# aehogan/lammps-induced-dipole-polarization-pair-style

Hardware: AMD Instinct MI355X
Metric: atom-steps/sec (higher is better)
Workload: dtype f64

## Files before the change

### include/polar_mi355x.h

```cpp
#ifndef POLAR_MI355X_H
#define POLAR_MI355X_H

#ifdef __cplusplus
extern "C" {
#endif

#define POLAR_OK 0
#define POLAR_WARN_NOT_CONVERGED 1
#define POLAR_RETRY_STEP 2
#define POLAR_ERR_INPUT -1
#define POLAR_ERR_NO_DEVICE -2
#define POLAR_ERR_HIP -3
#define POLAR_ERR_UNSUPPORTED -4
#define POLAR_ERR_STATE -5

enum { POLAR_DAMP_EXPONENTIAL = 0, POLAR_DAMP_NONE = 1 };

typedef struct polar_handle polar_handle;

typedef struct {
  double cut_lj_global, cut_coul;
  double polar_precision, polar_damp, polar_gamma;
  int iterations_max, damping_type, zodid, fixed_iteration;
  int polar_gs, polar_gs_ranked, use_previous, debug;
// ... 12 lines not shown
#define POLAR_ACCEL_MAX 8

typedef struct {
  double eng_vdwl, eng_coul, eng_pol;
  double u_self, u_ef, u_dd;
  double virial[6];
  double rmin;
  double rms_dmu;
  int iterations;
  int sweeps;
  int status;
  int ncolors;
  double ms_total, ms_rank, ms_ljcoul, ms_static, ms_solve, ms_force, ms_list;
  long long dd_pairs;
  double ms_color_host;
  double ms_kspace;
  int nkvec;
} polar_result;

int polar_create(int device, polar_handle **out);
int polar_destroy(polar_handle *h);
const char *polar_last_error(const polar_handle *h);
const char *polar_last_warning(const polar_handle *h);
int polar_device_count(void);
const char *polar_kernel_version(void);

int polar_pair_settings(polar_handle *h, int narg, const char *const *arg);
int polar_pair_coeff(polar_handle *h, int ntypes, int narg, const char *const *arg);
int polar_pair_modify(polar_handle *h, int narg, const char *const *arg);
int polar_pair_init(polar_handle *h, double g_ewald, double qqrd2e, const double special_lj[4],
                    const double special_coul[4]);
double polar_pair_cut(const polar_handle *h, int itype, int jtype);
double polar_pair_single(const polar_handle *h, double qi, double qj, int itype, int jtype, double rsq,
                         double factor_coul, double factor_lj, double *fforce);
const void *polar_pair_extract(const polar_handle *h, const char *name, int *dim);
int polar_get_settings(const polar_handle *h, polar_settings *out);

int polar_restart_pack(const polar_handle *h, void *buf, int max_bytes);
int polar_restart_unpack(polar_handle *h, const void *buf, int nbytes);
#define POLAR_RESTART_HEADER_BYTES 12

int polar_set_settings(polar_handle *h, const polar_settings *s);
int polar_set_types(polar_handle *h, int ntypes, const double *lj1, const double *lj2, const double *lj3,
                    const double *lj4, const double *offset, const double *cut_ljsq, const double *cutsq);
int polar_set_coul(polar_handle *h, double g_ewald, double qqrd2e, const double special_lj[4],
                   const double special_coul[4], int ncoultablebits, int ncoulmask, int ncoulshiftbits,
                   double tabinnersq, const double *rtable, const double *drtable, const double *ftable,
                   const double *dftable, const double *ctable, const double *dctable, const double *etable,
                   const double *detable);

int polar_set_box(polar_handle *h, const double boxlo[3], const double prd[3], const double tilt[3],
                  const int periodic[3], int triclinic);
int polar_set_atoms(polar_handle *h, int nlocal, int nghost, const double *x, const double *q,
                    const double *alpha, const int *type, const int *molecule);
int polar_set_positions(polar_handle *h, int nlocal, int nghost, const double *x);
int polar_set_positions_range(polar_handle *h, int lo, int hi, const double *x);
int polar_set_neighbors(polar_handle *h, int inum, const int *ilist, const int *numneigh,
                        int *const *firstneigh);
int polar_set_neighbors_csr(polar_handle *h, int inum, const int *ilist, const int *numneigh,
                            const long long *firstneigh, const int *neigh);

int polar_set_newton(polar_handle *h, int newton_pair);

int polar_build_neighbors(polar_handle *h, const double *cutneighsq, const int *tag, const int *nspecial,
                          const int *special, int maxspecial, const int special_flag[4],
                          int exclude_molecule_intra);

int polar_compute(polar_handle *h, int eflag, int vflag, double *f, double *mu, double *ef_static,
                  polar_result *out);
int polar_compute_peratom(polar_handle *h, int eflag, int vflag, double *f, double *mu, double *ef_static,
                          double *eatom, double *vatom, polar_result *out);

int polar_get_debug_trace(polar_handle *h, double *u_polar, int max);

int polar_get_debug_forces(polar_handle *h, double *out6);

int polar_get_colors(polar_handle *h, int *color, int n);

int polar_set_colors(polar_handle *h, const int *color, int n);

int polar_compute_resident(polar_handle *h, int eflag, int vflag, polar_result *out);
void *polar_dev_ptr(polar_handle *h, const char *name);
int polar_download(polar_handle *h, const char *name, double *dst, long long n);
int polar_upload_mu(polar_handle *h, const double *mu, long long n);


int polar_set_stream(polar_handle *h, void *hip_stream);
int polar_set_row_range(polar_handle *h, int lo, int hi);
int polar_set_global_count(polar_handle *h, long long natoms);
int polar_set_list_style(polar_handle *h, int full);
int polar_step_begin(polar_handle *h, int eflag, int vflag);
int polar_step_sweep(polar_handle *h);
int polar_step_sweep_phase(polar_handle *h, int color, int part);
int polar_step_sweep_part(polar_handle *h, int part, int nparts);
int polar_step_sweep_end(polar_handle *h, const double *dev_global_change);
int polar_step_sweep_end_n(polar_handle *h, const double *dev_global_change, int count);
int polar_step_state(polar_handle *h, int *done, int *iterations, int *status);
int polar_step_finish(polar_handle *h, polar_result *out);
int polar_mu_gather(polar_handle *h, long long lo, long long hi, double *dev_dst);
int polar_mu_scatter(polar_handle *h, long long lo, long long hi, const double *dev_src);
int polar_mu_gather_idx(polar_handle *h, const int *dev_idx, long long n, double *dev_dst);
int polar_mu_scatter_idx(polar_handle *h, const int *dev_idx, long long n, const double *dev_src);
int polar_change_export(polar_handle *h, double *dev_dst);
int polar_step_mu_get(polar_handle *h, long long lo, long long hi, double *mu_host);
int polar_step_mu_put_idx(polar_handle *h, long long n, const int *idx_host, const double *mu_host);
int polar_step_change_get(polar_handle *h, double *sum);
int polar_step_sweep_end_host(polar_handle *h, double global_change);

#define POLAR_DIST_ID_BYTES 128
typedef struct polar_dist polar_dist;
int polar_dist_unique_id(void *id128);
int polar_dist_create(const void *id128, int rank, int nranks, int device, polar_dist **out);
int polar_dist_destroy(polar_dist *d);
const char *polar_dist_last_error(const polar_dist *d);
int polar_dist_comm_count(const polar_dist *d);
int polar_dist_set_cadence(polar_dist *d, int reduce_every, int check_every);
int polar_dist_set_schedule(polar_dist *d, int lag, int my_class, int nclasses);
int polar_dist_set_halo(polar_dist *d, polar_handle *h, int npeers, const int *peers, const int *send_count, const int *send_idx,
                        const int *recv_count, const int *recv_idx);
int polar_dist_set_ghosts(polar_dist *d, polar_handle *h, int nghost, const int *owner, const double *shift);
int polar_dist_positions(polar_dist *d, polar_handle *h);
int polar_dist_exchange(polar_dist *d, polar_handle *h);
int polar_dist_step(polar_dist *d, polar_handle *h, int eflag, int vflag, polar_result *out);
int polar_dist_local_result(const polar_dist *d, polar_result *out);
int polar_dist_counters(const polar_dist *d, int *exchanges, int *allreduces);
#define POLAR_DIST_PROF_PARTS 5
int polar_dist_profile(polar_dist *d, int enable);
int polar_dist_profile_get(const polar_dist *d, double *ms_by_part, int *intervals);

#ifdef __cplusplus
}
#endif
#endif
```

### lammps-induced-dipole-polarization-pair-style_amd/__init__.py

```python
from __future__ import annotations

import ctypes as C
import importlib
import os
import subprocess

import numpy as np

_HERE = os.path.dirname(os.path.abspath(__file__))
_CSRC = os.path.join(_HERE, "csrc")
LIB_PATH = os.path.join(_HERE, "libpolar_mi355x.so")
LIB_PATH_LAB = os.path.join(_HERE, "libpolar_mi355x_lab.so")
HIPCC = os.environ.get("HIPCC", "/opt/rocm/bin/hipcc")
HIP_FLAGS = ["--offload-arch=gfx950", "-O3", "-std=c++17", "-fPIC", "-shared"]

_lib = None
_lib_lab = None


class PolarError(RuntimeError):

    def __init__(self, code, message):
        super().__init__(message)
        self.code = code
# ... 14 lines not shown
def build(force=False, verbose=False, lab=True):
    from concurrent.futures import ThreadPoolExecutor

    jobs, links = [], []
    for path, extra, tag in ((LIB_PATH, [], "product"), (LIB_PATH_LAB, ["-DPOLAR_LAB"], "lab")):
        if path == LIB_PATH_LAB and not lab:
            continue
        stale = (not os.path.exists(path)) or any(os.path.getmtime(s) > os.path.getmtime(path) for s in _sources(lab=(path == LIB_PATH_LAB)))
        if not (force or stale):
            continue
        odir = os.path.join(_CSRC, "build", tag)
        os.makedirs(odir, exist_ok=True)
        objs = []
        for tu in TRANSLATION_UNITS:
            obj = os.path.join(odir, tu.replace(".hip", ".o"))
            objs.append(obj)
            jobs.append([HIPCC] + [f for f in HIP_FLAGS if f != "-shared"] + extra + ["-Wno-unused-function", "-c", "-o", obj, os.path.join(_CSRC, tu)])
        links.append([HIPCC, "--offload-arch=gfx950", "-fPIC", "-shared", "-o", path] + objs)

    def run(cmd):
        if verbose:
            print(" ".join(cmd), flush=True)
        subprocess.check_call(cmd)

    if jobs:
        with ThreadPoolExecutor(max_workers=min(len(jobs), max(1, (os.cpu_count() or 2)))) as ex:
            list(ex.map(run, jobs))
        for cmd in links:
            run(cmd)
    return LIB_PATH


class Settings(C.Structure):
    _fields_ = [("cut_lj_global", C.c_double), ("cut_coul", C.c_double), ("polar_precision", C.c_double),
                ("polar_damp", C.c_double), ("polar_gamma", C.c_double), ("iterations_max", C.c_int),
                ("damping_type", C.c_int), ("zodid", C.c_int), ("fixed_iteration", C.c_int), ("polar_gs", C.c_int),
                ("polar_gs_ranked", C.c_int), ("use_previous", C.c_int), ("debug", C.c_int), ("dd_cutoff", C.c_double),
                ("device_neigh", C.c_int), ("restart_polar", C.c_int), ("deterministic", C.c_int), ("polar_sor", C.c_double), ("rccl_halo", C.c_int), ("polar_accel", C.c_int),
                ("polar_ewald", C.c_double)]


class Result(C.Structure):
    _fields_ = [("eng_vdwl", C.c_double), ("eng_coul", C.c_double), ("eng_pol", C.c_double), ("u_self", C.c_double),
                ("u_ef", C.c_double), ("u_dd", C.c_double), ("virial", C.c_double * 6), ("rmin", C.c_double),
                ("rms_dmu", C.c_double), ("iterations", C.c_int), ("sweeps", C.c_int), ("status", C.c_int),
                ("ncolors", C.c_int), ("ms_total", C.c_double), ("ms_rank", C.c_double), ("ms_ljcoul", C.c_double),
                ("ms_static", C.c_double), ("ms_solve", C.c_double), ("ms_force", C.c_double), ("ms_list", C.c_double),
                ("dd_pairs", C.c_longlong), ("ms_color_host", C.c_double), ("ms_kspace", C.c_double), ("nkvec", C.c_int)]


_dp, _ip, _llp = C.POINTER(C.c_double), C.POINTER(C.c_int), C.POINTER(C.c_longlong)
_cpp = C.POINTER(C.c_char_p)
EXPORTS = {
    "polar_create": (C.c_int, [C.c_int, C.POINTER(C.c_void_p)]),
    "polar_destroy": (C.c_int, [C.c_void_p]),
    "polar_last_error": (C.c_char_p, [C.c_void_p]),
    "polar_last_warning": (C.c_char_p, [C.c_void_p]),
    "polar_device_count": (C.c_int, []),
    "polar_kernel_version": (C.c_char_p, []),
    "polar_pair_settings": (C.c_int, [C.c_void_p, C.c_int, _cpp]),
    "polar_pair_coeff": (C.c_int, [C.c_void_p, C.c_int, C.c_int, _cpp]),
    "polar_pair_modify": (C.c_int, [C.c_void_p, C.c_int, _cpp]),
    "polar_pair_init": (C.c_int, [C.c_void_p, C.c_double, C.c_double, _dp, _dp]),
    "polar_pair_cut": (C.c_double, [C.c_void_p, C.c_int, C.c_int]),
    "polar_pair_single": (C.c_double, [C.c_void_p, C.c_double, C.c_double, C.c_int, C.c_int, C.c_double, C.c_double,
                                       C.c_double, _dp]),
    "polar_pair_extract": (C.c_void_p, [C.c_void_p, C.c_char_p, _ip]),
    "polar_get_settings": (C.c_int, [C.c_void_p, C.POINTER(Settings)]),
    "polar_set_settings": (C.c_int, [C.c_void_p, C.POINTER(Settings)]),
    "polar_set_types": (C.c_int, [C.c_void_p, C.c_int] + [_dp] * 7),
    "polar_set_coul": (C.c_int, [C.c_void_p, C.c_double, C.c_double, _dp, _dp, C.c_int, C.c_int, C.c_int, C.c_double]
                       + [_dp] * 8),
    "polar_set_box": (C.c_int, [C.c_void_p, _dp, _dp, _dp, _ip, C.c_int]),
    "polar_set_atoms": (C.c_int, [C.c_void_p, C.c_int, C.c_int, _dp, _dp, _dp, _ip, _ip]),
    "polar_set_positions": (C.c_int, [C.c_void_p, C.c_int, C.c_int, _dp]),
    "polar_set_neighbors": (C.c_int, [C.c_void_p, C.c_int, _ip, _ip, C.POINTER(_ip)]),
    "polar_set_neighbors_csr": (C.c_int, [C.c_void_p, C.c_int, _ip, _ip, _llp, _ip]),
    "polar_build_neighbors": (C.c_int, [C.c_void_p, _dp, _ip, _ip, _ip, C.c_int, _ip, C.c_int]),
    "polar_compute": (C.c_int, [C.c_void_p, C.c_int, C.c_int, _dp, _dp, _dp, C.POINTER(Result)]),
    "polar_compute_peratom": (C.c_int, [C.c_void_p, C.c_int, C.c_int, _dp, _dp, _dp, _dp, _dp, C.POINTER(Result)]),
    "polar_compute_resident": (C.c_int, [C.c_void_p, C.c_int, C.c_int, C.POINTER(Result)]),
    "polar_dev_ptr": (C.c_void_p, [C.c_void_p, C.c_char_p]),
    "polar_download": (C.c_int, [C.c_void_p, C.c_char_p, _dp, C.c_longlong]),
    "polar_upload_mu": (C.c_int, [C.c_void_p, _dp, C.c_longlong]),
    "polar_set_stream": (C.c_int, [C.c_void_p, C.c_void_p]),
    "polar_set_row_range": (C.c_int, [C.c_void_p, C.c_int, C.c_int]),
    "polar_set_global_count": (C.c_int, [C.c_void_p, C.c_longlong]),
    "polar_step_mu_get": (C.c_int, [C.c_void_p, C.c_longlong, C.c_longlong, _dp]),
    "polar_step_mu_put_idx": (C.c_int, [C.c_void_p, C.c_longlong, _ip, _dp]),
    "polar_step_change_get": (C.c_int, [C.c_void_p, _dp]),
    "polar_step_sweep_end_host": (C.c_int, [C.c_void_p, C.c_double]),
    "polar_step_sweep_end_n": (C.c_int, [C.c_void_p, C.c_void_p, C.c_int]),
    "polar_set_list_style": (C.c_int, [C.c_void_p, C.c_int]),
    "polar_set_newton": (C.c_int, [C.c_void_p, C.c_int]),
    "polar_get_debug_trace": (C.c_int, [C.c_void_p, _dp, C.c_int]),
    "polar_get_debug_forces": (C.c_int, [C.c_void_p, _dp]),
    "polar_get_colors": (C.c_int, [C.c_void_p, C.POINTER(C.c_int), C.c_int]),
    "polar_restart_pack": (C.c_int, [C.c_void_p, C.c_void_p, C.c_int]),
    "polar_restart_unpack": (C.c_int, [C.c_void_p, C.c_void_p, C.c_int]),
    "polar_step_begin": (C.c_int, [C.c_void_p, C.c_int, C.c_int]),
    "polar_step_sweep": (C.c_int, [C.c_void_p]),
    "polar_step_sweep_part": (C.c_int, [C.c_void_p, C.c_int, C.c_int]),
    "polar_step_sweep_end": (C.c_int, [C.c_void_p, C.c_void_p]),
    "polar_step_state": (C.c_int, [C.c_void_p, _ip, _ip, _ip]),
    "polar_step_finish": (C.c_int, [C.c_void_p, C.POINTER(Result)]),
    "polar_mu_gather": (C.c_int, [C.c_void_p, C.c_longlong, C.c_longlong, C.c_void_p]),
    "polar_mu_scatter": (C.c_int, [C.c_void_p, C.c_longlong, C.c_longlong, C.c_void_p]),
    "polar_mu_gather_idx": (C.c_int, [C.c_void_p, C.c_void_p, C.c_longlong, C.c_void_p]),
    "polar_mu_scatter_idx": (C.c_int, [C.c_void_p, C.c_void_p, C.c_longlong, C.c_void_p]),
    "polar_change_export": (C.c_int, [C.c_void_p, C.c_void_p]),
    "polar_dist_unique_id": (C.c_int, [C.c_void_p]),
    "polar_dist_create": (C.c_int, [C.c_void_p, C.c_int, C.c_int, C.c_int, C.POINTER(C.c_void_p)]),
    "polar_dist_destroy": (C.c_int, [C.c_void_p]),
    "polar_dist_last_error": (C.c_char_p, [C.c_void_p]),
    "polar_dist_set_cadence": (C.c_int, [C.c_void_p, C.c_int, C.c_int]),
    "polar_dist_set_halo": (C.c_int, [C.c_void_p, C.c_void_p, C.c_int, _ip, _ip, _ip, _ip, _ip]),
    "polar_dist_set_schedule": (C.c_int, [C.c_void_p, C.c_int, C.c_int, C.c_int]),
    "polar_dist_set_ghosts": (C.c_int, [C.c_void_p, C.c_void_p, C.c_int, _ip, _dp]),
    "polar_dist_positions": (C.c_int, [C.c_void_p, C.c_void_p]),
    "polar_dist_local_result": (C.c_int, [C.c_void_p, C.POINTER(Result)]),
    "polar_dist_comm_count": (C.c_int, [C.c_void_p]),
    "polar_step_sweep_phase": (C.c_int, [C.c_void_p, C.c_int, C.c_int]),
    "polar_set_colors": (C.c_int, [C.c_void_p, _ip, C.c_int]),
    "polar_set_positions_range": (C.c_int, [C.c_void_p, C.c_int, C.c_int, _dp]),
    "polar_dist_exchange": (C.c_int, [C.c_void_p, C.c_void_p]),
    "polar_dist_step": (C.c_int, [C.c_void_p, C.c_void_p, C.c_int, C.c_int, C.POINTER(Result)]),
    "polar_dist_counters": (C.c_int, [C.c_void_p, _ip, _ip]),
    "polar_dist_profile": (C.c_int, [C.c_void_p, C.c_int]),
    "polar_dist_profile_get": (C.c_int, [C.c_void_p, _dp, _ip]),
}


def lib(lab=False):
    global _lib, _lib_lab
    if lab:
        if _lib_lab is None:
            if not os.path.exists(LIB_PATH_LAB):
                raise PolarError(-2, f"{LIB_PATH_LAB} is missing: run __graft_entry__.build()")
            lib()
            L = C.CDLL(LIB_PATH_LAB)
            for name, (res, args) in EXPORTS.items():
                fn = getattr(L, name)
                fn.restype, fn.argtypes = res, args
            _lib_lab = L
        return _lib_lab
    if _lib is None:
        if not os.path.exists(LIB_PATH):
            raise PolarError(-2, f"{LIB_PATH} is missing: run __graft_entry__.build() (hipcc, gfx950); "
                                 "there is no CPU fallback for the polarization hot path")
        try:
            import torch
        except ImportError:
            pass
        L = C.CDLL(LIB_PATH)
        for name, (res, args) in EXPORTS.items():
            fn = getattr(L, name)
            fn.restype, fn.argtypes = res, args
        _lib = L
    return _lib


def device_count():
    return lib().polar_device_count()


def kernel_version():
# ... 172 lines not shown
        if getattr(st, "polar_accel", 0):
            args += ["polar_accel", str(int(st.polar_accel))]
        if getattr(st, "polar_ewald", 0.0):
            args += ["polar_ewald", repr(float(st.polar_ewald))]
        self.settings(args)
        if modify_args:
            self.modify(list(modify_args))
        return args

    def set_system(self, sysm):
        self._ck(self.L.polar_set_newton(self.h, int(sysm.extra.get("newton_pair", 1))))
        self.set_box(sysm.boxlo, sysm.prd, tilt=getattr(sysm, "tilt", (0.0, 0.0, 0.0)),
                     triclinic=int(getattr(sysm, "triclinic", 0)))
        self.set_atoms(sysm.nlocal, sysm.nghost, sysm.x, sysm.q, sysm.alpha, sysm.type, sysm.molecule)
        self.set_neighbors_csr(sysm.ilist, sysm.numneigh, sysm.firstneigh, sysm.neigh)

    def build_neighbors(self, cutneighsq, tag=None, nspecial=None, special=None, special_flag=(1, 2, 2, 2),
                        exclude_molecule_intra=False):
        cn = np.ascontiguousarray(cutneighsq, dtype=np.float64)
        keep = [cn]
        ip = lambda a: None if a is None else (keep.append(np.ascontiguousarray(a, dtype=np.int32)) or
                                               keep[-1].ctypes.data_as(_ip))
        sf = np.ascontiguousarray(special_flag, dtype=np.int32)
        maxspecial = 0 if special is None else int(np.asarray(special).shape[1])
        self._ck(self.L.polar_build_neighbors(self.h, _dptr(cn), ip(tag), ip(nspecial), ip(special), maxspecial,
                                              sf.ctypes.data_as(_ip), int(bool(exclude_molecule_intra))))

    def build_neighbors_from_system(self, sysm, skin=None):
        wlm = importlib.import_module(__name__ + ".workload")
        w = sysm.ntypes + 1
        cutneigh = sysm.extra["cutneigh"] if skin is None else float(np.sqrt(sysm.tables["cutsq"][1:, 1:].max())) + skin
        cn = np.full((w, w), cutneigh * cutneigh)
        nsp = sp = None
        if sysm.extra.get("special"):
            nsp, sp = wlm.lammps_special_arrays(sysm.nlocal, sysm.extra["special"])
        tag = (np.asarray(sysm.owner) + 1).astype(np.int32)
        self.build_neighbors(cn, tag, nsp, sp, wlm.neighbor_special_flag(sysm.special_lj, sysm.special_coul),
                             sysm.extra.get("exclude_intra", False))

    def compute(self, eflag=1, vflag=2, mu=None, want_ef=True):
        n, nall = self.nlocal, self.nlocal + self.nghost
        f = np.zeros((nall, 3))
        mu = np.zeros((n, 3)) if mu is None else np.array(mu, dtype=np.float64, copy=True)
        ef = np.zeros((n, 3))
        res = Result()
        eatom = vatom = None
        if eflag // 2 or vflag // 4:
            eatom = np.zeros(nall) if eflag // 2 else None
            vatom = np.zeros((nall, 6)) if vflag // 4 else None
            rc = self._ck(self.L.polar_compute_peratom(
                self.h, eflag, vflag, _dptr(f), _dptr(mu), _dptr(ef) if want_ef else None,
                _dptr(eatom) if eatom is not None else None, _dptr(vatom) if vatom is not None else None,
                C.byref(res)))
        else:
            rc = self._ck(self.L.polar_compute(self.h, eflag, vflag, _dptr(f), _dptr(mu),
                                               _dptr(ef) if want_ef else None, C.byref(res)))
        out = _result_dict(res)
        out.update(f=f, mu=mu, ef_static=ef, status=rc, warning=self.L.polar_last_warning(self.h).decode(),
                   eatom=eatom, vatom=vatom)
        return out

    def compute_resident(self, eflag=1, vflag=2):
        res = Result()
        rc = self._ck(self.L.polar_compute_resident(self.h, eflag, vflag, C.byref(res)))
        out = _result_dict(res)
        out.update(status=rc, warning=self.L.polar_last_warning(self.h).decode())
        return out

    def debug_trace(self, nmax=1024):
        a = np.zeros(nmax)
        n = self._ck(self.L.polar_get_debug_trace(self.h, _dptr(a), nmax))
        return a[:n].copy()

    def debug_forces(self):
        a = np.zeros(6)
        self._ck(self.L.polar_get_debug_forces(self.h, _dptr(a)))
        return a[:3].copy(), a[3:].copy()

    def colors(self, n):
        a = np.full(n, -1, dtype=np.int32)
        nc = self._ck(self.L.polar_get_colors(self.h, a.ctypes.data_as(C.POINTER(C.c_int)), n))
        return nc, a

    def download(self, name, n):
        a = np.zeros(n)
        self._ck(self.L.polar_download(self.h, name.encode(), _dptr(a), n))
        return a


class PolarDist:

    @staticmethod
    def unique_id():
        buf = C.create_string_buffer(128)
        rc = lib().polar_dist_unique_id(buf)
        if rc < 0:
            raise PolarError(rc, "polar_dist_unique_id failed (is RCCL available?)")
        return buf.raw

    def __init__(self, unique_id, rank, nranks, device=0):
        self.L = lib()
        self.d = C.c_void_p()
        self.rank, self.nranks = rank, nranks
        rc = self.L.polar_dist_create(C.c_char_p(bytes(unique_id)), rank, nranks, device, C.byref(self.d))
        if rc < 0:
            raise PolarError(rc, self.L.polar_dist_last_error(self.d).decode())

    def _ck(self, rc):
        if rc < 0:
            raise PolarError(rc, self.L.polar_dist_last_error(self.d).decode())
        return rc

    def set_cadence(self, reduce_every=1, check_every=4):
        self._ck(self.L.polar_dist_set_cadence(self.d, reduce_every, check_every))

    def set_halo(self, pair, peers, send_lists, recv_lists):
        peers = np.ascontiguousarray(peers, dtype=np.int32)
        sc = np.array([len(a) for a in send_lists], dtype=np.int32)
        rc_ = np.array([len(a) for a in recv_lists], dtype=np.int32)
        si = np.ascontiguousarray(np.concatenate([np.asarray(a, dtype=np.int32) for a in send_lists]) if len(send_lists) else np.zeros(0, np.int32))
        ri = np.ascontiguousarray(np.concatenate([np.asarray(a, dtype=np.int32) for a in recv_lists]) if len(recv_lists) else np.zeros(0, np.int32))
        self._ck(self.L.polar_dist_set_halo(self.d, pair.h, len(peers), _iptr(peers), _iptr(sc), _iptr(si) if len(si) else None,
                                            _iptr(rc_), _iptr(ri) if len(ri) else None))

    def set_schedule(self, lag=1, my_class=0, nclasses=0):
        self._ck(self.L.polar_dist_set_schedule(self.d, lag, my_class, nclasses))

    def set_ghosts(self, pair, owner, shift):
        owner = np.ascontiguousarray(owner, dtype=np.int32)
        shift = np.ascontiguousarray(shift, dtype=np.float64)
        self._ck(self.L.polar_dist_set_ghosts(self.d, pair.h, len(owner), _iptr(owner) if len(owner) else None, _dptr(shift) if len(owner) else None))

    def positions(self, pair):
        self._ck(self.L.polar_dist_positions(self.d, pair.h))

    def local_result(self):
        res = Result()
        self._ck(self.L.polar_dist_local_result(self.d, C.byref(res)))
        return _result_dict(res)

    def comm_count(self):
        return self._ck(self.L.polar_dist_comm_count(self.d))

    PROFILE_PARTS = ("other", "sweep_kernels", "stop_rule", "exchange", "accel")

    def profile(self, enable=True):
        self._ck(self.L.polar_dist_profile(self.d, 1 if enable else 0))

    def profile_get(self):
        ms = (C.c_double * len(self.PROFILE_PARTS))()
        n = C.c_int()
        self._ck(self.L.polar_dist_profile_get(self.d, ms, C.byref(n)))
        out = {k: float(v) for k, v in zip(self.PROFILE_PARTS, ms)}
        out["intervals"] = n.value
        return out

    def exchange(self, pair):
        self._ck(self.L.polar_dist_exchange(self.d, pair.h))

    def step(self, pair, eflag=1, vflag=2):
        res = Result()
        rc = self._ck(self.L.polar_dist_step(self.d, pair.h, eflag, vflag, C.byref(res)))
        out = _result_dict(res)
        ex, ar = C.c_int(), C.c_int()
        self.L.polar_dist_counters(self.d, C.byref(ex), C.byref(ar))
        out.update(status=rc, warning=pair.L.polar_last_warning(pair.h).decode(), exchanges=ex.value, allreduces=ar.value)
# ... 38 lines not shown
```

### lammps-induced-dipole-polarization-pair-style_amd/csrc/lab/lists_cluster_rows.hpp

```cpp
struct ClusterRows {
  const int4 *members;
  int ncl;
};
static __global__ __launch_bounds__(POLAR_BLOCK) void k_cl_build(ClusterRows cl, const double4 *__restrict__ pos4, Box box,
                                                          CellGrid g, const long long *__restrict__ cell_first,
                                                          double ddcutsq, long long pitch, int *__restrict__ cnt,
                                                          int *__restrict__ dd_j, int pad_index,
                                                          int *__restrict__ wrapf, int *__restrict__ overflow,
                                                          unsigned long long *__restrict__ total) {
  const int lane = threadIdx.x & 63;
  const int c = blockIdx.x * POLAR_ROWS_PER_BLOCK + (threadIdx.x >> 6);
  if (c >= cl.ncl) return;
  const int4 mem = cl.members[c];
  const int m0 = __builtin_amdgcn_readfirstlane(mem.x), m1 = __builtin_amdgcn_readfirstlane(mem.y),
            m2 = __builtin_amdgcn_readfirstlane(mem.z), m3 = __builtin_amdgcn_readfirstlane(mem.w);
  double mx[4], my[4], mz[4];
  const int mi[4] = {m0, m1, m2, m3};
#pragma unroll
  for (int k = 0; k < 4; k++) {
    const double4 r = pos4[mi[k] >= 0 ? mi[k] : m0];
    mx[k] = wave_uniform(r.x); my[k] = wave_uniform(r.y); mz[k] = wave_uniform(r.z);
  }
  double rmax2 = 0.0;
#pragma unroll
  for (int k = 1; k < 4; k++) {
    double ex, ey, ez;
    min_image_rint(box, mx[0], my[0], mz[0], mx[k], my[k], mz[k], ex, ey, ez);
    const double d2 = ex * ex + ey * ey + ez * ez;
    rmax2 = (mi[k] >= 0 && d2 > rmax2) ? d2 : rmax2;
  }
  const double reach = wave_uniform(sqrt(ddcutsq) + sqrt(rmax2) + 1e-6);
  const double reach2 = reach * reach;
  int cc[3], W[3];
  double uu[3], edge[3];
  {
    double fr3[3];
    frac_coords(box, g.lo, mx[0], my[0], mz[0], fr3);
#pragma unroll
    for (int k = 0; k < 3; k++) {
      double fr = fr3[k];
      fr -= floor(fr);
      const double t = fr * g.nc[k];
      int ck = (int)t;
      ck = ck >= g.nc[k] ? g.nc[k] - 1 : ck;
      cc[k] = __builtin_amdgcn_readfirstlane(ck);
      uu[k] = wave_uniform(t - ck); edge[k] = wave_uniform(box.prd[k] / g.nc[k]);
      int w = (int)ceil(reach / edge[k]);
      W[k] = __builtin_amdgcn_readfirstlane(w < 1 ? 1 : (w > 3 ? 3 : w));
    }
  }
  const int c0 = cc[0], c1 = cc[1], c2 = cc[2];
  const long long row0 = (long long)c * pitch;
  const unsigned long long below = (lane == 0) ? 0ull : (~0ull >> (64 - lane));
  const int n0 = g.nc[0], n1 = g.nc[1], n2 = g.nc[2];
  const bool f2 = n2 >= 2 * W[2] + 1, f1 = n1 >= 2 * W[1] + 1, f0 = n0 >= 2 * W[0] + 1;
  const int zlo = f2 ? c2 - W[2] : 0, zcnt = f2 ? 2 * W[2] + 1 : n2;
  const int ylo = f1 ? c1 - W[1] : 0, ycnt = f1 ? 2 * W[1] + 1 : n1;
  const int nsr = zcnt * ycnt;
  int ra0 = 0, rb0 = 0, ra1 = 0, rb1 = 0;
  if (lane < nsr) {
    const int zz = zlo + lane / ycnt, yy = ylo + lane % ycnt;
    int b2 = zz, b1 = yy;
    bool ok = true;
    if (b2 < 0 || b2 >= n2) { if (!box.periodic[2]) ok = false; b2 = (b2 + n2) % n2; }
    if (b1 < 0 || b1 >= n1) { if (!box.periodic[1]) ok = false; b1 = (b1 + n1) % n1; }
    double dzmin = 0.0, dymin = 0.0;
    if (f2) { const int d = zz - c2; dzmin = d > 0 ? (d - uu[2]) * edge[2] : (d < 0 ? (uu[2] - (d + 1)) * edge[2] : 0.0); }
    if (f1) { const int d = yy - c1; dymin = d > 0 ? (d - uu[1]) * edge[1] : (d < 0 ? (uu[1] - (d + 1)) * edge[1] : 0.0); }
    const double rem2 = reach2 - dzmin * dzmin - dymin * dymin;
    if (rem2 < 0.0) ok = false;
    int xlo = f0 ? c0 - W[0] : 0, xhi = f0 ? c0 + W[0] : n0 - 1;
    if (ok && f0) {
      const double xr = sqrt(rem2) / edge[0];
      int lo_off = (int)floor(uu[0] - xr), hi_off = (int)floor(uu[0] + xr);
      lo_off = lo_off < -W[0] ? -W[0] : lo_off; hi_off = hi_off > W[0] ? W[0] : hi_off;
      xlo = c0 + lo_off; xhi = c0 + hi_off;
    }
    if (ok) {
      const long long rowbase = ((long long)b2 * n1 + b1) * n0;
      const int xa = xlo < 0 ? 0 : xlo, xb = xhi >= n0 ? n0 - 1 : xhi;
      ra0 = (int)cell_first[rowbase + xa]; rb0 = (int)cell_first[rowbase + xb + 1];
      if (box.periodic[0]) {
        if (xlo < 0) { ra1 = (int)cell_first[rowbase + xlo + n0]; rb1 = (int)cell_first[rowbase + n0]; }
        else if (xhi >= n0) { ra1 = (int)cell_first[rowbase]; rb1 = (int)cell_first[rowbase + xhi - n0 + 1]; }
      }
    }
  }
  int count = 0;
  unsigned long long anywrap = 0ull, npairs = 0ull;
  for (int sr = 0; sr < nsr; sr++) {
#pragma unroll
    for (int piece = 0; piece < 2; piece++) {
      const int a = __builtin_amdgcn_readlane(piece ? ra1 : ra0, sr), b = __builtin_amdgcn_readlane(piece ? rb1 : rb0, sr);
      for (int base = a; base < b; base += 64) {
        const int j = base + lane;
        bool in = false, wr = false;
        int hits = 0;
        if (j < b && j != m0 && j != m1 && j != m2 && j != m3) {
          const double4 rj = pos4[j];
          if (__double2loint(rj.w)) {
#pragma unroll
            for (int k = 0; k < 4; k++) {
              double ex, ey, ez;
              min_image_rint(box, mx[k], my[k], mz[k], rj.x, rj.y, rj.z, ex, ey, ez);
              const bool hit = mi[k] >= 0 && (ex * ex + ey * ey + ez * ez) < ddcutsq;
              hits += hit;
              wr |= hit && (ex != mx[k] - rj.x || ey != my[k] - rj.y || ez != mz[k] - rj.z);
            }
            in = hits > 0;
          }
        }
        const unsigned long long m_in = __ballot(in);
        anywrap |= __ballot(wr);
        const int kd = count + __popcll(m_in & below);
        if (in && kd < pitch) dd_j[row0 + lp_slot(kd)] = j << 6;
        count += __popcll(m_in);
        npairs += (unsigned long long)hits;
      }
    }
  }
  const int have = count < pitch ? count : (int)pitch;
  const int padded = (have + 63) & ~63;
  for (int k = have + lane; k < padded; k += 64) dd_j[row0 + lp_slot(k)] = pad_index << 6;
  double np = (double)npairs;
  np = wave_sum(np);
  if (lane == 0) {
    cnt[c] = count;
    wrapf[c] = anywrap != 0ull;
    if (count > pitch) atomicMax(overflow, count);
    if (np > 0.0) atomicAdd(total + (blockIdx.x & 63) * 16, (unsigned long long)np);
  }
}
```

### lammps-induced-dipole-polarization-pair-style_amd/csrc/lab/lists_paired_rows.hpp

```cpp
struct PhaseOff { int n; int off[66]; };
__device__ __forceinline__ int phase_of(const PhaseOff &P, int r) {
  int q = 0;
  while (q + 1 < P.n && r >= P.off[q + 1]) q++;
  return q;
}
static __global__ void k_unit_flag(int ntot, const int *__restrict__ rows, const int *__restrict__ perm, const int *__restrict__ cell_id,
                            PhaseOff P, int *__restrict__ lead) {
  const int r = blockIdx.x * blockDim.x + threadIdx.x;
  if (r >= ntot) return;
  const int q = phase_of(P, r);
  const int lo = P.off[q];
  const int c = cell_id[perm[rows ? rows[r] : r]];
  int k = 0;
  for (int b = r - 1; b >= lo && cell_id[perm[rows ? rows[b] : b]] == c; b--) k++;
  lead[r] = (k & 1) ? 0 : 1;
}
static __global__ void k_unit_fill(int ntot, const int *__restrict__ rows, const int *__restrict__ perm, const int *__restrict__ cell_id,
                            PhaseOff P, const int *__restrict__ lead, const long long *__restrict__ upos, int2 *__restrict__ unit) {
  const int r = blockIdx.x * blockDim.x + threadIdx.x;
  if (r >= ntot || !lead[r]) return;
  const int q = phase_of(P, r);
  const int hi = P.off[q + 1];
  const int iA = rows ? rows[r] : r;
  int iB = -1;
  if (r + 1 < hi) {
    const int cand = rows ? rows[r + 1] : r + 1;
    if (cell_id[perm[cand]] == cell_id[perm[iA]]) iB = cand;
  }
  unit[upos[r]] = make_int2(iA, iB);
}
template <bool TRI>
static __global__ __launch_bounds__(POLAR_BLOCK) void k_dd_units(int nunits, const int2 *__restrict__ unit, const double4 *__restrict__ pos4,
                                                          Box box, CellGrid g, const long long *__restrict__ cell_first, double ddcutsq,
                                                          long long upitch, int *__restrict__ udd_j, int4 *__restrict__ udesc, int qm,
                                                          int dummy, int *__restrict__ overflow, unsigned long long *__restrict__ dd_total) {
  const int lane = threadIdx.x & 63;
  const int u = blockIdx.x * POLAR_ROWS_PER_BLOCK + (threadIdx.x >> 6);
  if (u >= nunits) return;
  const int2 un = unit[u];
  const int iA = un.x, iB = un.y;
  const double4 rA = pos4[iA];
  const double4 rB = pos4[iB >= 0 ? iB : iA];
  int cc[3];
  {
    double fr3[3];
    frac_coords(box, g.lo, rA.x, rA.y, rA.z, fr3);
#pragma unroll
    for (int k = 0; k < 3; k++) {
      double fr = fr3[k];
      fr -= floor(fr);
      int ck = (int)(fr * g.nc[k]);
      ck = ck >= g.nc[k] ? g.nc[k] - 1 : ck;
      cc[k] = __builtin_amdgcn_readfirstlane(ck);
    }
  }
  const int c0 = cc[0], c1 = cc[1], c2 = cc[2];
  const long long d0 = (long long)u * upitch;
  const unsigned long long below = (lane == 0) ? 0ull : (~0ull >> (64 - lane));
  const int n0 = g.nc[0], n1 = g.nc[1], n2 = g.nc[2];
  const int zlo = n2 >= 5 ? c2 - 2 : 0, zcnt = n2 >= 5 ? 5 : n2;
  const int ylo = n1 >= 5 ? c1 - 2 : 0, ycnt = n1 >= 5 ? 5 : n1;
  const int nsr = zcnt * ycnt;
  int ra0 = 0, rb0 = 0, ra1 = 0, rb1 = 0;
  if (lane < nsr) {
    const int zz = zlo + lane / ycnt, yy = ylo + lane % ycnt;
    int b2 = zz, b1 = yy;
    bool ok = true;
    if (b2 < 0 || b2 >= n2) { if (!box.periodic[2]) ok = false; b2 = (b2 + n2) % n2; }
    if (b1 < 0 || b1 >= n1) { if (!box.periodic[1]) ok = false; b1 = (b1 + n1) % n1; }
    const int xlo = n0 >= 5 ? c0 - 2 : 0, xhi = n0 >= 5 ? c0 + 2 : n0 - 1;
    if (ok) {
      const long long rowbase = ((long long)b2 * n1 + b1) * n0;
      const int xa = xlo < 0 ? 0 : xlo, xb = xhi >= n0 ? n0 - 1 : xhi;
      ra0 = (int)cell_first[rowbase + xa]; rb0 = (int)cell_first[rowbase + xb + 1];
      if (box.periodic[0]) {
        if (xlo < 0) { ra1 = (int)cell_first[rowbase + xlo + n0]; rb1 = (int)cell_first[rowbase + n0]; }
        else if (xhi >= n0) { ra1 = (int)cell_first[rowbase]; rb1 = (int)cell_first[rowbase + xhi - n0 + 1]; }
      }
    }
  }
  int count = 0, useful = 0;
  bool wrap_lane = false;
  for (int sr = 0; sr < nsr; sr++) {
#pragma unroll
    for (int piece = 0; piece < 2; piece++) {
      const int a = __builtin_amdgcn_readlane(piece ? ra1 : ra0, sr), b = __builtin_amdgcn_readlane(piece ? rb1 : rb0, sr);
      for (int base = a; base < b; base += 64) {
        const int j = base + lane;
        bool inA = false, inB = false;
        if (j < b) {
          const double4 rj = pos4[j];
          if (__double2loint(rj.w)) {
            double ex, ey, ez;
            const bool shA = min_image_rint_w<TRI>(box, rA.x, rA.y, rA.z, rj.x, rj.y, rj.z, ex, ey, ez);
            inA = j != iA && ex * ex + ey * ey + ez * ez < ddcutsq;
            bool shB = false;
            if (iB >= 0) {
              shB = min_image_rint_w<TRI>(box, rB.x, rB.y, rB.z, rj.x, rj.y, rj.z, ex, ey, ez);
              inB = j != iB && ex * ex + ey * ey + ez * ez < ddcutsq;
            }
            wrap_lane |= (inA && shA) || (inB && shB);
          }
        }
        const bool in = inA || inB;
        const unsigned long long m = __ballot(in);
        const int k = count + __popcll(m & below);
        if (in && k < upitch) udd_j[d0 + lp_slot(k, qm)] = (j << 6) | (inA ? 1 : 0) | (inB ? 2 : 0);
        count += __popcll(m);
        useful += __popcll(__ballot(inA)) + __popcll(__ballot(inB));
      }
    }
  }
  const int have = count < upitch ? count : (int)upitch;
  const int padded = (have + 63) & ~63;
  for (int k = have + lane; k < padded; k += 64) udd_j[d0 + lp_slot(k, qm)] = dummy << 6;
  const unsigned long long anywrap = __ballot(wrap_lane);
  if (lane == 0) {
    udesc[u] = make_int4(iA, iB, (padded >> 6) | (anywrap ? 0x40000000 : 0), count);
    if (count > upitch) atomicMax(overflow, count);
    if (useful) atomicAdd(dd_total + (blockIdx.x & 63) * 16, (unsigned long long)useful);
  }
}
```

### lammps-induced-dipole-polarization-pair-style_amd/csrc/polar_api.hip

```cpp
#include "polar_handle.hpp"

namespace {
void upload_types(polar_handle *h, int ntypes, const double *const t[7]) {
  need_device(h);
  const size_t m = (size_t)(ntypes + 1) * (ntypes + 1);
  std::vector<double> pack(8 * m, 0.0);
  for (size_t k = 0; k < m; k++) {
    pack[8 * k + 0] = t[6][k]; pack[8 * k + 1] = t[5][k]; pack[8 * k + 2] = t[0][k]; pack[8 * k + 3] = t[1][k];
    pack[8 * k + 4] = t[2][k]; pack[8 * k + 5] = t[3][k]; pack[8 * k + 6] = t[4][k];
  }
  h->d_lj.ensure(8 * m);
  HIPCHECK(hipMemcpy(h->d_lj.p, pack.data(), 8 * m * sizeof(double), hipMemcpyHostToDevice));
  h->P.ntypes = ntypes;
  h->P.ljpack = h->d_lj.p;
  h->ntypes = ntypes;
  h->types_set = true;
}

void upload_coul(polar_handle *h, double g_ewald, double qqrd2e, const double *slj, const double *scoul, int nbits,
                 int mask, int shift, double tabinnersq, const double *const t[8]) {
  need_device(h);
  h->P.g_ewald = g_ewald; h->P.qqrd2e = qqrd2e;
  for (int k = 0; k < 4; k++) { h->P.special_lj[k] = slj[k]; h->P.special_coul[k] = scoul[k]; }
  h->P.ncoultablebits = nbits; h->P.ncoulmask = mask; h->P.ncoulshiftbits = shift; h->P.tabinnersq = tabinnersq;
// ... 81 lines not shown
      HIPCHECK(hipHostMalloc((void **)&p, (size_t)CH * sizeof(int)));
      HIPCHECK(hipEventCreateWithFlags(&e, hipEventDisableTiming));
      h->h_nl_stage.push_back(p); h->ev_nl.push_back(e);
    }
    if (chunk >= kRing) HIPCHECK(hipEventSynchronize(h->ev_nl[buf]));
    int *dst = h->h_nl_stage[buf];
    const long long t0 = at[ii0], cnt = at[ii1] - t0;
    pool.run([&](int part) {
      const long long lo = t0 + cnt * part / nt, hi = t0 + cnt * (part + 1) / nt;
      int a = (int)(std::lower_bound(at.begin() + ii0, at.begin() + ii1, lo) - at.begin());
      const int b = (int)(std::lower_bound(at.begin() + ii0, at.begin() + ii1, hi) - at.begin());
      int worst = 0;
      for (; a < b; a++) {
        const int i = ilist[a], m = numneigh[i];
        const int *src = row(i);
        int *d = dst + (at[a] - t0);
        int mx = 0;
        for (int k = 0; k < m; k++) { const int v = src[k]; d[k] = v; const int j = v & 0x3FFFFFFF; mx = j > mx ? j : mx; }
        worst = mx > worst ? mx : worst;
      }
      if (worst >= nall) bad[(size_t)part * 16] = 1;
    }, nt);
    for (int t = 0; t < nt; t++) if (bad[(size_t)t * 16]) { HIPCHECK(hipStreamSynchronize(s)); throw InputError("neighbor index out of range"); }
    if (cnt > 0) HIPCHECK(hipMemcpyAsync(h->d_neigh.p + t0, dst, (size_t)cnt * sizeof(int), hipMemcpyHostToDevice, s));
    HIPCHECK(hipEventRecord(h->ev_nl[buf], s));
    ii0 = ii1; chunk++;
  }
  HIPCHECK(hipEventRecord(h->ev_list_up, s));
  h->list_up_pending = true;
  h->neigh_set = true;
  h->sym_valid = false;
  if (h->colors_valid) h->colors_recheck = true;
  h->device_list = false;
  h->full_list = h->user_full_list;
}
}


extern "C" {

const char *polar_kernel_version(void) { return POLAR_KERNEL_VERSION; }

int polar_device_count(void) {
  int n = 0;
  if (hipGetDeviceCount(&n) != hipSuccess) return 0;
  return n;
}

int polar_create(int device, polar_handle **out) {
  if (!out) return POLAR_ERR_STATE;
  polar_handle *h = new polar_handle();
  *out = h;
  h->device = device;
  if (const char *e = getenv("POLAR_COLOR_DIST")) h->color_dist = atof(e);
  h->color_keep = std::max(h->color_dist - 0.4, 0.75 * h->color_dist);
  if (const char *e = getenv("POLAR_COLOR_KEEP")) h->color_keep = atof(e);
  if (const char *e = getenv("POLAR_DETERMINISTIC")) h->deterministic = atoi(e) != 0;
#ifdef POLAR_LAB
#include "lab/api_env_knobs.inc"
#endif
  int n = polar_device_count();
  if (n <= 0 || device < 0 || device >= n) {
    h->have_device = false;
    h->err = "no usable HIP device";
    return POLAR_OK;
  }
  return guarded(h, [&]() {
    HIPCHECK(hipSetDevice(device));
    HIPCHECK(hipStreamCreate(&h->stream));
    for (auto &e : h->ev) HIPCHECK(hipEventCreate(&e));
    {
      int prio_lo = 0, prio_hi = 0;
      HIPCHECK(hipDeviceGetStreamPriorityRange(&prio_lo, &prio_hi));
      HIPCHECK(hipStreamCreateWithPriority(&h->lj_stream, hipStreamNonBlocking, prio_lo));
    }
    HIPCHECK(hipEventCreate(&h->ev_fork)); HIPCHECK(hipEventCreate(&h->ev_join));
    HIPCHECK(hipEventCreate(&h->ev_lj0)); HIPCHECK(hipEventCreate(&h->ev_lj1));
    HIPCHECK(hipEventCreateWithFlags(&h->ev_dl0, hipEventDisableTiming)); HIPCHECK(hipEventCreateWithFlags(&h->ev_dl1, hipEventDisableTiming));
    HIPCHECK(hipEventCreateWithFlags(&h->ev_mu_ready, hipEventDisableTiming));
    for (auto &e : h->ev_fchunk) HIPCHECK(hipEventCreateWithFlags(&e, hipEventDisableTiming));
    for (auto &e : h->ev_ks) HIPCHECK(hipEventCreate(&e));
    HIPCHECK(hipStreamCreateWithFlags(&h->dl_stream, hipStreamNonBlocking));
    if (getenv("POLAR_NO_OVERLAP")) h->overlap_lj = false;
    if (const char *e = getenv("POLAR_LJ_PERS")) h->lj_pers = atoi(e);
    if (const char *e = getenv("POLAR_LJ_PERS_THREADS")) h->lj_pers_threads = std::max(256, std::min(POLAR_LJ_PERS_THREADS, (atoi(e) / 64) * 64));
    { int ncu = 0; if (hipDeviceGetAttribute(&ncu, hipDeviceAttributeMultiprocessorCount, device) == hipSuccess) h->ncu = ncu; }
    HIPCHECK(hipHostMalloc((void **)&h->h_scal, sizeof(Scal)));
    HIPCHECK(hipHostMalloc((void **)&h->h_flags, 16 * sizeof(int)));
    HIPCHECK(hipHostMalloc((void **)&h->h_ddtot, 64 * 16 * sizeof(unsigned long long)));
    h->d_overflow.ensure(16); h->d_ddtot.ensure(64 * 16);
    h->d_scal.ensure(1);
    h->d_slots.ensure((size_t)POLAR_NSLOT * POLAR_SLOT_STRIDE);
    h->have_device = true;
    return POLAR_OK;
  });
}

int polar_destroy(polar_handle *h) {
  if (!h) return POLAR_OK;
  if (h->have_device) {
    (void)hipSetDevice(h->device);
    (void)hipStreamSynchronize(h->stream);
    if (h->lj_stream) { (void)hipStreamSynchronize(h->lj_stream); (void)hipStreamDestroy(h->lj_stream); }
    for (hipEvent_t e : {h->ev_fork, h->ev_join, h->ev_lj0, h->ev_lj1, h->ev_dl0, h->ev_dl1, h->ev_mu_ready}) if (e) (void)hipEventDestroy(e);
    for (hipEvent_t e : h->ev_ks) if (e) (void)hipEventDestroy(e);
    if (h->dl_stream) (void)hipStreamDestroy(h->dl_stream);
    if (h->up_stream) { (void)hipStreamSynchronize(h->up_stream); (void)hipStreamDestroy(h->up_stream); }
    if (h->ev_list_up) (void)hipEventDestroy(h->ev_list_up);
    for (int *p : h->h_nl_stage) (void)hipHostFree(p);
    for (hipEvent_t e : h->ev_nl) (void)hipEventDestroy(e);
    for (hipEvent_t e : h->ev_fchunk) if (e) (void)hipEventDestroy(e);
    h->d_ljpos.release(); h->d_ljaux.release(); h->d_tag.release(); h->d_nspecial.release(); h->d_special.release();
    h->d_ljcell_id.release(); h->d_ljcell_cnt.release(); h->d_ljcell_fill.release(); h->d_ljcell_first.release(); h->d_cutneighsq.release();
    h->d_xchg.release(); h->d_xidx.release();
    h->d_eatom.release(); h->d_vatom.release(); h->d_dd_r2.release(); h->d_fpol.release();
    h->d_x.release(); h->d_q.release(); h->d_alpha.release(); h->d_f.release(); h->d_ef.release(); h->d_F.release();
    h->d_mu.release(); h->d_mu0.release(); h->d_acc_x.release(); h->d_acc_f.release(); h->d_acc_g.release(); h->d_acc_dF.release(); h->d_acc_dG.release(); h->d_acc_part.release(); h->d_acc_state.release(); h->d_bflag.release(); h->d_rank.release(); h->d_dmu.release(); h->d_tab.release(); h->d_lj.release();
    h->d_type.release(); h->d_mol.release(); h->d_order.release(); h->d_pos.release(); h->d_ilist.release();
    h->d_numneigh.release(); h->d_neigh.release(); h->d_rows.release(); h->d_first.release();
    h->d_sym_first.release(); h->d_sym_cnt.release(); h->d_sym_fill.release(); h->d_sym_j.release();
    h->d_mol_s.release(); h->d_perm.release(); h->d_inv.release(); h->d_rows_orig.release(); h->d_ownrows.release(); h->d_ef_s.release(); h->d_scan_a.release(); h->d_scan_b.release(); h->d_gs_cnt.release(); h->d_T6.release(); h->d_Minv.release(); h->d_gsN.release(); h->d_gsAT.release(); h->d_cb.release(); h->d_gs_part.release();
    h->d_rec0.release(); h->d_rec1.release(); h->d_scal.release(); h->d_slots.release();
    h->d_cell_id.release(); h->d_cell_cnt.release(); h->d_cell_fill.release();
    h->d_nl_cnt.release(); h->d_dd_cnt.release(); h->d_dd_wrap.release(); h->d_lpdesc.release(); h->d_slot.release(); h->d_color_orig.release(); h->d_color_s.release(); h->d_trace.release(); h->d_ew_kv.release(); h->d_ew_hkl.release(); h->d_ew_rows.release(); h->d_ew_s.release(); h->d_ew_m.release(); h->d_ew_part.release(); h->d_ew_erec.release(); h->d_ew_vpart.release(); h->d_ew_out.release(); h->d_cl_orig.release(); h->d_cl_cnt.release(); h->d_cl_wrap.release(); h->d_cl_tw.release(); h->d_cl_s.release(); h->d_nl_j.release(); h->d_dd_j.release();
    h->d_cell_first.release(); h->d_nl_first.release(); h->d_dd_first.release(); h->d_dd_s.release(); h->d_xq.release(); h->d_pos4.release();
    h->d_overflow.release(); h->d_ddtot.release();
    h->d_cadj.release(); h->d_cdeg.release(); h->d_ccnt.release(); h->d_cflags.release(); h->d_crelabel.release(); h->d_klist.release(); h->d_dbgf.release(); h->d_ulead.release(); h->d_udd_j.release(); h->d_upos.release(); h->d_unit.release(); h->d_udesc.release(); h->d_cprio.release(); h->d_cstat.release(); h->d_coff.release(); h->d_lp_pend.release(); h->d_lp_part.release();
    if (h->h_cflags) (void)hipHostFree(h->h_cflags);
    if (h->h_cstat) (void)hipHostFree(h->h_cstat);
    if (h->h_coff) (void)hipHostFree(h->h_coff);
    h->d_srec0.release(); h->d_srec1.release(); h->d_thdr.release(); h->d_trow.release(); h->d_un_j.release(); h->d_dd16.release(); h->d_pend.release();
    if (h->h_flags) (void)hipHostFree(h->h_flags);
    if (h->h_ddtot) (void)hipHostFree(h->h_ddtot);
    if (h->h_scal) (void)hipHostFree(h->h_scal);
    if (h->h_stage) (void)hipHostFree(h->h_stage);
    for (auto &e : h->ev) if (e) (void)hipEventDestroy(e);
    if (h->stream && h->own_stream) (void)hipStreamDestroy(h->stream);
  }
  delete h;
  return POLAR_OK;
}

const char *polar_last_error(const polar_handle *h) { return h ? h->err.c_str() : "null handle"; }
const char *polar_last_warning(const polar_handle *h) { return h ? h->warn.c_str() : ""; }

int polar_pair_settings(polar_handle *h, int narg, const char *const *arg) {
  return guarded(h, [&]() { h->ph.settings(narg, arg); h->colors_valid = false; h->nl_pitch = h->dd_pitch = 0; h->cl_pitch = 0; h->un_pitch = 0; h->pitch16 = 0; return POLAR_OK; });
}
int polar_pair_coeff(polar_handle *h, int ntypes, int narg, const char *const *arg) {
  return guarded(h, [&]() { h->ph.coeff(ntypes, narg, arg); return POLAR_OK; });
}
int polar_pair_modify(polar_handle *h, int narg, const char *const *arg) {
  return guarded(h, [&]() { h->ph.modify(narg, arg); return POLAR_OK; });
}
int polar_pair_init(polar_handle *h, double g_ewald, double qqrd2e, const double special_lj[4],
                    const double special_coul[4]) {
  return guarded(h, [&]() {
    PairHost &p = h->ph;
    p.init(g_ewald, qqrd2e, special_lj, special_coul);
    h->coul_set = false;
    if (h->have_device) {
      HIPCHECK(hipSetDevice(h->device));
      const double *t[7] = {p.lj1.data(), p.lj2.data(), p.lj3.data(), p.lj4.data(), p.offset.data(), p.cut_ljsq.data(), p.cutsq.data()};
      upload_types(h, p.ntypes, t);
      if (p.ncoultablebits == 0) {
        const double *c[8];
// ... 391 lines not shown
    h->early_ef = ef_static ? st + 3 * nall + 3 * n : nullptr;
    h->user_mu = mu; h->user_ef = ef_static;
    const bool dbg = getenv("POLAR_DEBUG") != nullptr;
    auto t0 = std::chrono::steady_clock::now();
    auto lap = [&](const char *what) {
      if (!dbg) return;
      const auto t1 = std::chrono::steady_clock::now();
      fprintf(stderr, "[polar] compute: %-22s %7.3f ms\n", what, std::chrono::duration<double, std::milli>(t1 - t0).count());
      t0 = t1;
    };
    int rc = do_compute(h, eflag, vflag, mu, out);
    if (rc < 0) return rc;
    lap("device step + sync");
    const size_t tot = 3 * nall, piece = (tot + 3) / 4;
    for (int k = 0; k < 4; k++) {
      const size_t a = std::min(tot, k * piece), b = std::min(tot, (k + 1) * piece);
      if (b > a) HIPCHECK(hipMemcpyAsync(st + a, h->d_f.p + a, (b - a) * sizeof(double), hipMemcpyDeviceToHost, h->stream));
      HIPCHECK(hipEventRecord(h->ev_fchunk[k], h->stream));
    }
    for (int k = 0; k < 4; k++) {
      const size_t a = std::min(tot, k * piece), b = std::min(tot, (k + 1) * piece);
      HIPCHECK(hipEventSynchronize(h->ev_fchunk[k]));
      host_chunks(b - a, [&](size_t lo, size_t hi) { for (size_t i = a + lo; i < a + hi; i++) f[i] += st[i]; });
    }
    lap("f arrived and added");
    h->mu_host_in_sync = true;
    return rc;
  });
}

int polar_compute_peratom(polar_handle *h, int eflag, int vflag, double *f, double *mu, double *ef_static,
                          double *eatom, double *vatom, polar_result *out) {
  return guarded(h, [&]() {
    if (!f || !mu || !out) throw std::runtime_error("polar_compute_peratom: null output pointer");
    if ((eflag / 2 && !eatom) || (vflag / 4 && !vatom)) throw InputError("polar_compute_peratom: eflag & 2 needs eatom, vflag & 4 needs vatom");
    need_device(h);
    HIPCHECK(hipSetDevice(h->device));
    int rc = do_compute(h, eflag, vflag, mu, out);
    if (rc < 0) return rc;
    const size_t n = h->nlocal, nall = (size_t)h->nlocal + h->nghost;
    auto add_from = [&](const double *dev, double *host, size_t cnt) {
      h->h_tmp.resize(cnt);
      HIPCHECK(hipMemcpy(h->h_tmp.data(), dev, cnt * sizeof(double), hipMemcpyDeviceToHost));
      for (size_t k = 0; k < cnt; k++) host[k] += h->h_tmp[k];
    };
    add_from(h->d_f.p, f, 3 * nall);
    if (eflag / 2) add_from(h->d_eatom.p, eatom, nall);
    if (vflag / 4) add_from(h->d_vatom.p, vatom, 6 * nall);
    HIPCHECK(hipMemcpy(mu, h->d_mu.p, 3 * n * sizeof(double), hipMemcpyDeviceToHost));
    if (ef_static) HIPCHECK(hipMemcpy(ef_static, h->d_ef.p, 3 * n * sizeof(double), hipMemcpyDeviceToHost));
    h->mu_host_in_sync = true;
    return rc;
  });
}

int polar_compute_resident(polar_handle *h, int eflag, int vflag, polar_result *out) {
  return guarded(h, [&]() {
    if (!out) throw std::runtime_error("polar_compute_resident: null result pointer");
    need_device(h);
    HIPCHECK(hipSetDevice(h->device));
    return do_compute(h, eflag, vflag, nullptr, out);
  });
}

void *polar_dev_ptr(polar_handle *h, const char *name) {
  if (!h || !name || !h->have_device) return nullptr;
  if (strcmp(name, "f") == 0) return h->d_f.p;
  if (strcmp(name, "mu") == 0) return h->d_mu.p;
  if (strcmp(name, "ef_static") == 0) return h->d_ef.p;
  if (strcmp(name, "x") == 0) return h->d_x.p;
  if (strcmp(name, "eatom") == 0) return h->d_eatom.p;
  if (strcmp(name, "vatom") == 0) return h->d_vatom.p;
  return nullptr;
}
int polar_download(polar_handle *h, const char *name, double *dst, long long n) {
  return guarded(h, [&]() {
    need_device(h);
    void *p = polar_dev_ptr(h, name);
    if (!p) throw std::runtime_error("polar_download: unknown array name");
    HIPCHECK(hipMemcpy(dst, p, (size_t)n * sizeof(double), hipMemcpyDeviceToHost));
    return POLAR_OK;
  });
}
int polar_upload_mu(polar_handle *h, const double *mu, long long n) {
  return guarded(h, [&]() {
    need_device(h);
    h->d_mu.ensure((size_t)n);
    HIPCHECK(hipMemcpy(h->d_mu.p, mu, (size_t)n * sizeof(double), hipMemcpyHostToDevice));
    h->mu_resident = true;
    return POLAR_OK;
  });
}

int polar_set_stream(polar_handle *h, void *hip_stream) {
  return guarded(h, [&]() {
    need_device(h);
    if (h->own_stream && h->stream) { HIPCHECK(hipStreamSynchronize(h->stream)); HIPCHECK(hipStreamDestroy(h->stream)); }
    h->stream = (hipStream_t)hip_stream;
    h->own_stream = false;
    return POLAR_OK;
  });
}
int polar_set_row_range(polar_handle *h, int lo, int hi) {
  return guarded(h, [&]() {
    if (lo < 0 || (hi >= 0 && hi < lo)) throw InputError("bad row range");
    h->row_lo = lo; h->row_hi = hi;
    return POLAR_OK;
  });
}
int polar_set_global_count(polar_handle *h, long long natoms) {
  if (!h) return POLAR_ERR_STATE;
  if (natoms < 0 || natoms > 2147483647LL) return fail(h, POLAR_ERR_INPUT, "bad global atom count");
  h->global_count = natoms;
  return POLAR_OK;
}
int polar_get_debug_trace(polar_handle *h, double *u_polar, int max) {
  if (!h) return POLAR_ERR_STATE;
  int n = 0;
  int rc = guarded(h, [&]() {
    need_device(h);
    n = std::min(h->ntrace, max);
    if (n > 0) HIPCHECK(hipMemcpy(u_polar, h->d_trace.p, (size_t)n * sizeof(double), hipMemcpyDeviceToHost));
    return (int)POLAR_OK;
  });
  return rc < 0 ? rc : n;
}
int polar_get_colors(polar_handle *h, int *color, int n) {
  if (!h) return POLAR_ERR_STATE;
  int nc = 0;
  int rc = guarded(h, [&]() {
    need_device(h);
    if (!color || n < 0) throw InputError("polar_get_colors: null pointer");
    const int m = std::min(n, h->nlocal);
    for (int k = 0; k < n; k++) color[k] = -1;
    if (!h->colors_valid || (int)h->color_off.size() < 2) return (int)POLAR_OK;
    nc = (int)h->color_off.size() - 1;
    if (h->d_color_orig.p && h->d_color_orig.cap >= (size_t)m && m > 0)
      HIPCHECK(hipMemcpy(color, h->d_color_orig.p, (size_t)m * sizeof(int), hipMemcpyDeviceToHost));
    return (int)POLAR_OK;
  });
  return rc < 0 ? rc : nc;
}
int polar_get_debug_forces(polar_handle *h, double *out6) {
  return guarded(h, [&]() {
    need_device(h);
    if (!out6) throw InputError("polar_get_debug_forces: null pointer");
    for (int k = 0; k < 6; k++) out6[k] = 0.0;
    if (!h->ph.st.debug || !h->d_dbgf.p) return 0;
    HIPCHECK(hipMemcpy(out6, h->d_dbgf.p, 6 * sizeof(double), hipMemcpyDeviceToHost));
    return 1;
  });
}
int polar_set_newton(polar_handle *h, int newton_pair) {
  if (!h) return POLAR_ERR_STATE;
  h->newton_pair = newton_pair ? 1 : 0;
  return POLAR_OK;
}
int polar_set_list_style(polar_handle *h, int full) {
  if (!h) return POLAR_ERR_STATE;
  h->user_full_list = full ? 1 : 0;
  if (!h->device_list) h->full_list = h->user_full_list;
  return POLAR_OK;
}
int polar_step_begin(polar_handle *h, int eflag, int vflag) {
  return guarded(h, [&]() {
    step_begin_lists(h, eflag, vflag);
// ... 200 lines not shown
```

### lammps-induced-dipole-polarization-pair-style_amd/csrc/polar_common.hpp

```cpp
#pragma once

#include <hip/hip_runtime.h>
#include <stdint.h>

#ifdef POLAR_LAB
#define POLAR_LAB_PARAM , int ablate
#define POLAR_LAB_PASS , ablate
#define POLAR_ABL(bit) (ablate & (bit))
#else
#define POLAR_LAB_PARAM
#define POLAR_LAB_PASS
#define POLAR_ABL(bit) 0
#endif

namespace polar {


struct __attribute__((aligned(64))) AtomRec {
  double x, mx;
  double y, my;
  double z, mz;
  double q, a;
};

// ... 116 lines not shown
  }
  ex = wrap_ci(ex, b.prd[0], b.half[0], b.periodic[0]);
  dx = -ex; dy = -ey; dz = -ez;
}

__device__ __forceinline__ double quad_xor(double v, const int which) {
  int lo = __double2loint(v), hi = __double2hiint(v);
  if (which == 1) {
    lo = __builtin_amdgcn_update_dpp(0, lo, 0xB1, 0xF, 0xF, true);
    hi = __builtin_amdgcn_update_dpp(0, hi, 0xB1, 0xF, 0xF, true);
  } else {
    lo = __builtin_amdgcn_update_dpp(0, lo, 0x4E, 0xF, 0xF, true);
    hi = __builtin_amdgcn_update_dpp(0, hi, 0x4E, 0xF, 0xF, true);
  }
  return __hiloint2double(hi, lo);
}
__device__ __forceinline__ double quad_sum(double v) {
  v += quad_xor(v, 1);
  v += quad_xor(v, 2);
  return v;
}

struct RowList {
  const int *cnt;
  long long pitch;
};
__device__ __forceinline__ void row_range(const RowList &L, int i, long long &beg, long long &end) {
  beg = (long long)i * L.pitch;
  const long long c = L.cnt[i];
  end = beg + (c < L.pitch ? c : L.pitch);
}

__device__ __forceinline__ void min_image_rint(const Box &b, double xi, double yi, double zi, double xj, double yj,
                                               double zj, double &dx, double &dy, double &dz) {
  double ex = xi - xj, ey = yi - yj, ez = zi - zj;
  const double nz = b.periodic[2] ? rint(ez * b.inv[2]) : 0.0;
  ez = fma(-b.prd[2], nz, ez); ey = fma(-b.yz, nz, ey); ex = fma(-b.xz, nz, ex);
  const double ny = b.periodic[1] ? rint(ey * b.inv[1]) : 0.0;
  ey = fma(-b.prd[1], ny, ey); ex = fma(-b.xy, ny, ex);
  const double nx = b.periodic[0] ? rint(ex * b.inv[0]) : 0.0;
  ex = fma(-b.prd[0], nx, ex);
  dx = ex; dy = ey; dz = ez;
}
template <bool TRI>
__device__ __forceinline__ bool min_image_rint_w(const Box &b, double xi, double yi, double zi, double xj, double yj,
                                                 double zj, double &dx, double &dy, double &dz) {
  double ex = xi - xj, ey = yi - yj, ez = zi - zj;
  const double nz = b.periodic[2] ? rint(ez * b.inv[2]) : 0.0;
  ez = fma(-b.prd[2], nz, ez);
  if (TRI) { ey = fma(-b.yz, nz, ey); ex = fma(-b.xz, nz, ex); }
  const double ny = b.periodic[1] ? rint(ey * b.inv[1]) : 0.0;
  ey = fma(-b.prd[1], ny, ey);
  if (TRI) ex = fma(-b.xy, ny, ex);
  const double nx = b.periodic[0] ? rint(ex * b.inv[0]) : 0.0;
  ex = fma(-b.prd[0], nx, ex);
  dx = ex; dy = ey; dz = ez;
  return nz != 0.0 || ny != 0.0 || nx != 0.0;
}
__host__ __device__ __forceinline__ void frac_coords(const Box &b, const double lo[3], double x, double y, double z, double fr[3]) {
  fr[2] = (z - lo[2]) * b.inv[2];
  if (b.triclinic) {
    fr[1] = ((y - lo[1]) - b.yz * fr[2] * 1.0) * b.inv[1];
    fr[0] = ((x - lo[0]) - b.xy * fr[1] - b.xz * fr[2]) * b.inv[0];
  } else {
    fr[1] = (y - lo[1]) * b.inv[1];
    fr[0] = (x - lo[0]) * b.inv[0];
  }
}
template <bool EXACT>
__device__ __forceinline__ void pair_del(const Box &b, double xi, double yi, double zi, double xj, double yj,
                                         double zj, double &dx, double &dy, double &dz) {
  if (EXACT) min_image_del(b, xi, yi, zi, xj, yj, zj, dx, dy, dz);
  else min_image_rint(b, xi, yi, zi, xj, yj, zj, dx, dy, dz);
}

__host__ __device__ __forceinline__ long long lp_slot(long long e, int qm = 1) {
  const long long p = e & 63;
  const long long lane = qm ? (((p & 15) << 2) | (p >> 4)) : p;
  return ((e >> 8) << 8) + (lane << 2) + ((e >> 6) & 3);
}

#define POLAR_NL_SAMEMOL 0x40000000
#define POLAR_NL_MASK 0x3FFFFFFF

struct RecQuad { double2 a, b, c, d; };
__device__ __forceinline__ RecQuad fetch_records(const AtomRec *__restrict__ rec, int j, double2 *stage, int lane) {
  const int q4 = lane >> 2;
  const char *base = reinterpret_cast<const char *>(rec);
  const unsigned piece = (unsigned)(lane & 3) * 16u, k = lane & 3;
  const unsigned j0 = __shfl(j, q4, 64), j1 = __shfl(j, 16 + q4, 64), j2 = __shfl(j, 32 + q4, 64), j3 = __shfl(j, 48 + q4, 64);
  const double2 p0 = *reinterpret_cast<const double2 *>(base + ((j0 << 6) + piece));
  const double2 p1 = *reinterpret_cast<const double2 *>(base + ((j1 << 6) + piece));
  const double2 p2 = *reinterpret_cast<const double2 *>(base + ((j2 << 6) + piece));
  const double2 p3 = *reinterpret_cast<const double2 *>(base + ((j3 << 6) + piece));
  stage[q4 * 5 + k] = p0; stage[(16 + q4) * 5 + k] = p1;
  stage[(32 + q4) * 5 + k] = p2; stage[(48 + q4) * 5 + k] = p3;
  __builtin_amdgcn_fence(__ATOMIC_RELEASE, "wavefront");
  __builtin_amdgcn_wave_barrier();
  __builtin_amdgcn_fence(__ATOMIC_ACQUIRE, "wavefront");
  RecQuad r;
  r.a = stage[lane * 5]; r.b = stage[lane * 5 + 1]; r.c = stage[lane * 5 + 2]; r.d = stage[lane * 5 + 3];
  __builtin_amdgcn_wave_barrier();
  return r;
}

struct XQ { double2 a, b; };
__device__ __forceinline__ XQ fetch_xq(const double4 *__restrict__ xq, int j, double2 *stage, int lane) {
  const int h2 = lane >> 1;
  const char *base = reinterpret_cast<const char *>(xq);
  const unsigned piece = (unsigned)(lane & 1) * 16u, k = lane & 1;
  const unsigned j0 = __shfl(j, h2, 64), j1 = __shfl(j, 32 + h2, 64);
  const double2 p0 = *reinterpret_cast<const double2 *>(base + ((j0 << 5) + piece));
  const double2 p1 = *reinterpret_cast<const double2 *>(base + ((j1 << 5) + piece));
  stage[h2 * 3 + k] = p0; stage[(32 + h2) * 3 + k] = p1;
  __builtin_amdgcn_fence(__ATOMIC_RELEASE, "wavefront");
  __builtin_amdgcn_wave_barrier();
  __builtin_amdgcn_fence(__ATOMIC_ACQUIRE, "wavefront");
  XQ r;
  r.a = stage[lane * 3]; r.b = stage[lane * 3 + 1];
  __builtin_amdgcn_wave_barrier();
  return r;
}

struct ExpCoef {
  double log2e, ln2hi, ln2lo;
  double c[14];
};
inline ExpCoef make_expcoef() {
  ExpCoef K;
  K.log2e = 1.4426950408889634074; K.ln2hi = 6.93147180369123816490e-01; K.ln2lo = 1.90821492927058770002e-10;
  const double c[14] = {1.0, 1.0, 0.5, 0.16666666666666666, 0.041666666666666664, 0.008333333333333333, 0.001388888888888889, 0.0001984126984126984, 2.48015873015873e-05, 2.7557319223985893e-06, 2.755731922398589e-07, 2.505210838544172e-08, 2.08767569878681e-09, 1.6059043836821613e-10};
  for (int k = 0; k < 14; k++) K.c[k] = c[k];
  return K;
}
__device__ __forceinline__ double exp_neg(double x, const ExpCoef &K) {
  x = fmax(x, -745.0);
  const double n = rint(x * K.log2e);
  double r = fma(-n, K.ln2hi, x);
  r = fma(-n, K.ln2lo, r);
  double p = K.c[13];
#pragma unroll
  for (int k = 12; k >= 0; k--) p = fma(p, r, K.c[k]);
  return ldexp(p, (int)n);
}
__device__ __forceinline__ double rsqrt_pos(double x) {
  const double y = __builtin_amdgcn_rsq(x);
  const double e = fma(-(x * y), y, 1.0);
  return fma(y * e, 0.5, y);
}
__device__ __forceinline__ double rsqrt_pos3(double x) {
  const double y = __builtin_amdgcn_rsq(x);
  const double e = fma(-(x * y), y, 1.0);
  return fma(y * e, fma(e, 0.375, 0.5), y);
}
template <int DEG = 10>
__device__ __forceinline__ double exp_neg_fast(double x, const ExpCoef &K) {
  static_assert(DEG >= 1 && DEG <= 13, "ExpCoef holds 1/k! up to k = 13");
  x = fmax(x, -700.0);
  const double shift = 6755399441055744.0;
  const double ns = fma(x, K.log2e, shift);
  const double n = ns - shift;
  double r = fma(-n, K.ln2hi, x);
  r = fma(-n, K.ln2lo, r);
  double p = K.c[DEG];
#pragma unroll
  for (int k = DEG - 1; k >= 0; k--) p = fma(p, r, K.c[k]);
// ... 57 lines not shown
```

### lammps-induced-dipole-polarization-pair-style_amd/csrc/polar_handle.hpp

```cpp
#pragma once
#include <hip/hip_runtime.h>

#include <algorithm>
#include <initializer_list>
#include <utility>
#include <chrono>
#include <cmath>
#include <cstdio>
#include <cstdlib>
#include <exception>
#include <cstring>
#include <numeric>
#include <string>
#include <thread>
#include <mutex>
#include <condition_variable>
#include <functional>
#include <memory>
#include <stdexcept>
#include <unistd.h>
#include <vector>

#include "pair_host.hpp"
#include "polar_kernels.hpp"
// ... 165 lines not shown
  long long slots_epoch = -1;
  bool colors_recheck = false;
  std::vector<int> h_color;
  DBuf<int> d_color_orig, d_color_s;
  DBuf<int> d_klist;
  DBuf<int> d_cadj, d_cdeg, d_ccnt, d_cflags, d_crelabel;
  DBuf<unsigned long long> d_cprio;
  DBuf<double> d_cstat;
  DBuf<long long> d_coff;
  int *h_cflags = nullptr;
  double *h_cstat = nullptr;
  long long *h_coff = nullptr;
  int cadj_pitch = 16;
  int host_colors = 0;
  int colors_reused = 0, colors_rebuilt = 0;
  double ms_color_host = 0.0;
  double color_dist = 2.4;
  int field_block = 256;
  double bbox_lo[3] = {0, 0, 0}, bbox_hi[3] = {0, 0, 0};
  long long global_count = 0;
  DBuf<double> d_xchg; DBuf<int> d_xidx;
  bool device_list = false;
  int user_full_list = 0;
  long long lj_pitch = 0;
  DBuf<double4> d_ljpos; DBuf<int2> d_ljaux; DBuf<int> d_tag, d_nspecial, d_special, d_ljcell_id, d_ljcell_cnt, d_ljcell_fill; DBuf<long long> d_ljcell_first; DBuf<double> d_cutneighsq;
  int lj_typed = 1;
  bool lj_tab_arith = false;
  int lj_pers = 1;
  int ncu = 0;
  int lj_pers_threads = 768;
  bool sym_typed = false, dev_typed = false;
  int static_xq = 1;
  int pol_first = 1;
#ifdef POLAR_LAB
  int force_literal = 0;
#endif
  int part_k = 0, part_n = 1;
  int lp_wg_per_cu = 0;
  int lp_quad_major = 1;
  int quad_block = POLAR_BLOCK;
  int lp_tiles = 2;
  int lp_rows = 1;
  int lp_pairs = 0;
  DBuf<int> d_ulead, d_udd_j;
  DBuf<long long> d_upos;
  DBuf<int2> d_unit;
  DBuf<int4> d_udesc;
  std::vector<int> unit_off;
  long long upitch = 0;
  int lp_depth = 0;
  int cache_r2 = -1;
  int stream_mode = 1;
  int sweep_kernel = 2;
  int ablate = 0;
  DBuf<SRec> d_srec0, d_srec1;
  DBuf<TileHdr> d_thdr;
  DBuf<TileRowEnt> d_trow;
  DBuf<int> d_un_j;
  DBuf<unsigned short> d_dd16;
  DBuf<double> d_pend;
  int un_pitch = 0;
  int un_lds = 0;
  long long pitch16 = 0;
  int tile_max_u = 0;
  bool tile_reported = false;
  double dens = 0.0;
  std::vector<TileLaunch> tile_launches;
  TileLaunch tile_all{};
  size_t tile_lds_attr[16] = {0, 0, 0, 0, 0, 0, 0, 0, 0, 0, 0, 0, 0, 0, 0, 0};
  size_t tile_build_lds_attr = 0;
  int tile_waves = 4;
  int tile_wide = 0;
  int tile_sw[3] = {2, 2, 2};
  int deterministic = 0;
  Scal *h_scal = nullptr;
  hipEvent_t ev[8] = {};
  hipStream_t lj_stream = nullptr;
  hipEvent_t ev_fork = nullptr, ev_join = nullptr, ev_lj0 = nullptr, ev_lj1 = nullptr, ev_dl0 = nullptr, ev_dl1 = nullptr;
  hipStream_t dl_stream = nullptr;
  hipEvent_t ev_mu_ready = nullptr;
  double *early_mu = nullptr, *early_ef = nullptr, *user_mu = nullptr, *user_ef = nullptr;
  hipEvent_t ev_fchunk[4] = {nullptr, nullptr, nullptr, nullptr};
  bool overlap_lj = true;
  bool lj_forked = false;
  std::vector<double> h_tmp;
  double *h_stage = nullptr;
  DBuf<double> d_trace;
  DBuf<double4> d_ew_kv; DBuf<int4> d_ew_hkl, d_ew_rows;
  DBuf<double2> d_ew_s, d_ew_m, d_ew_part;
  DBuf<double> d_ew_erec, d_ew_vpart, d_ew_out;
  std::vector<double> ew_key;
  int ew_nk = 0, ew_nrow = 0, ew_nm = 0;
  double ew_cell[6] = {0, 0, 0, 0, 0, 0};
  hipEvent_t ev_ks[4] = {nullptr, nullptr, nullptr, nullptr};
  int ntrace = 0;
  size_t h_stage_cap = 0;
};
inline int fail(polar_handle *h, int code, const std::string &m) {
  if (h) h->err = m;
  return code;
}

template <typename F>
int guarded(polar_handle *h, F &&fn) {
  if (!h) return POLAR_ERR_STATE;
  try {
    return fn();
  } catch (const InputError &e) {
    return fail(h, POLAR_ERR_INPUT, e.what());
  } catch (const Unsupported &e) {
    return fail(h, POLAR_ERR_UNSUPPORTED, e.what());
  } catch (const NoDevice &e) {
    return fail(h, POLAR_ERR_NO_DEVICE, e.what());
  } catch (const HipError &e) {
    return fail(h, POLAR_ERR_HIP, e.what());
  } catch (const std::exception &e) {
    return fail(h, POLAR_ERR_STATE, e.what());
  }
}

inline double *staging(polar_handle *h, size_t count) {
  if (count > h->h_stage_cap) {
    if (h->h_stage) {
      if (h->stream) (void)hipStreamSynchronize(h->stream);
      if (h->dl_stream) (void)hipStreamSynchronize(h->dl_stream);
      (void)hipHostFree(h->h_stage);
    }
    h->h_stage = nullptr; h->h_stage_cap = 0;
    const size_t want = count + count / 4 + 1024;
    HIPCHECK(hipHostMalloc((void **)&h->h_stage, want * sizeof(double)));
    h->h_stage_cap = want;
  }
  return h->h_stage;
}

inline void need_device(polar_handle *h) {
  if (!h->have_device) throw NoDevice();
}

class HostPool {
 public:
  static HostPool &get() { static HostPool p; return p; }
  int width() const { return (int)th_.size() + 1; }
  void run(const std::function<void(int)> &fn, int parts) {
    if (parts <= 1 || th_.empty() || getpid() != pid_) { for (int k = 0; k < parts; k++) fn(k); return; }
    std::unique_lock<std::mutex> job(job_m_);
    {
      std::lock_guard<std::mutex> g(m_);
      fn_ = &fn; parts_ = parts; pending_ = std::min(parts - 1, (int)th_.size()); gen_++; failed_ = nullptr;
    }
    cv_.notify_all();
    std::exception_ptr mine;
    try {
      fn(0);
      for (int k = (int)th_.size() + 1; k < parts; k++) fn(k);
    } catch (...) { mine = std::current_exception(); }
    std::unique_lock<std::mutex> g(m_);
    done_.wait(g, [&] { return pending_ == 0; });
    fn_ = nullptr;
    std::exception_ptr theirs = failed_;
    failed_ = nullptr;
    g.unlock();
    if (mine) std::rethrow_exception(mine);
    if (theirs) std::rethrow_exception(theirs);
  }
 private:
// ... 119 lines not shown
```

### lammps-induced-dipole-polarization-pair-style_amd/csrc/polar_lists.hpp

```cpp
#pragma once

#include "polar_common.hpp"

namespace polar {

struct CellGrid {
  int trim;
  int nc[3];
  double lo[3], inv[3];
};

__device__ __forceinline__ int cell_of(const CellGrid &g, const Box &b, double x, double y, double z) {
  int c[3];
  double fr3[3];
  frac_coords(b, g.lo, x, y, z, fr3);
#pragma unroll
  for (int k = 0; k < 3; k++) {
    double fr = fr3[k];
    fr -= floor(fr);
    int ck = (int)(fr * g.nc[k]);
    c[k] = ck >= g.nc[k] ? g.nc[k] - 1 : ck;
  }
  return (c[2] * g.nc[1] + c[1]) * g.nc[0] + c[0];
}

static __global__ void k_cell_count(int n, const double *__restrict__ x, CellGrid g, Box b, int *__restrict__ cell_id,
                             int *__restrict__ cell_cnt) {
  int i = blockIdx.x * blockDim.x + threadIdx.x;
  if (i >= n) return;
  int c = cell_of(g, b, x[3 * i], x[3 * i + 1], x[3 * i + 2]);
  cell_id[i] = c;
  atomicAdd(&cell_cnt[c], 1);
}

#define POLAR_SCAN_ITEMS 4096
static __global__ __launch_bounds__(1024) void k_scan_block(long long n, const int *__restrict__ in, long long *__restrict__ out,
                                                     long long *__restrict__ btot) {
  __shared__ long long wtot[16];
  const int t = threadIdx.x, lane = t & 63, wv = t >> 6;
  const long long base = (long long)blockIdx.x * POLAR_SCAN_ITEMS + 4 * t;
  int v[4] = {0, 0, 0, 0};
  if (base + 3 < n) { const int4 q = *(const int4 *)(in + base); v[0] = q.x; v[1] = q.y; v[2] = q.z; v[3] = q.w; }
  else for (int k = 0; k < 4; k++) if (base + k < n) v[k] = in[base + k];
  const long long s = (long long)v[0] + v[1] + v[2] + v[3];
  long long inc = s;
#pragma unroll
  for (int off = 1; off < 64; off <<= 1) {
    const long long up = __shfl_up(inc, off, 64);
    if (lane >= off) inc += up;
  }
  if (lane == 63) wtot[wv] = inc;
  __syncthreads();
  if (wv == 0) {
    long long x = lane < 16 ? wtot[lane] : 0, w = x;
#pragma unroll
    for (int off = 1; off < 16; off <<= 1) {
      const long long up = __shfl_up(w, off, 64);
      if (lane >= off) w += up;
    }
    if (lane < 16) wtot[lane] = w - x;
    if (lane == 15) { btot[blockIdx.x] = w; if (gridDim.x == 1) out[n] = w; }
  }
  __syncthreads();
  long long run = wtot[wv] + inc - s;
#pragma unroll
  for (int k = 0; k < 4; k++) { if (base + k < n) out[base + k] = run; run += v[k]; }
}
static __global__ __launch_bounds__(1024) void k_scan_totals(int nb, long long *__restrict__ btot, long long *__restrict__ total) {
  __shared__ long long wtot[16];
  __shared__ long long carry;
  const int t = threadIdx.x, lane = t & 63, wv = t >> 6;
  if (t == 0) carry = 0;
  __syncthreads();
  for (int b0 = 0; b0 < nb; b0 += 1024) {
    const long long s = b0 + t < nb ? btot[b0 + t] : 0;
    long long inc = s;
#pragma unroll
    for (int off = 1; off < 64; off <<= 1) {
      const long long up = __shfl_up(inc, off, 64);
      if (lane >= off) inc += up;
    }
    if (lane == 63) wtot[wv] = inc;
    __syncthreads();
    if (wv == 0) {
      long long x = lane < 16 ? wtot[lane] : 0, w = x;
#pragma unroll
      for (int off = 1; off < 16; off <<= 1) {
        const long long up = __shfl_up(w, off, 64);
        if (lane >= off) w += up;
      }
      if (lane < 16) wtot[lane] = w - x;
    }
// ... 4 lines not shown
    if (t == 1023) carry = mine + s;
    __syncthreads();
  }
  if (t == 0) *total = carry;
}
static __global__ __launch_bounds__(256) void k_scan_add(long long n, long long *__restrict__ out, const long long *__restrict__ boff) {
  const long long i = (long long)blockIdx.x * 256 + threadIdx.x + POLAR_SCAN_ITEMS;
  if (i < n) out[i] += boff[i / POLAR_SCAN_ITEMS];
}

static __global__ void k_cell_fill(int n, const int *__restrict__ cell_id, const long long *__restrict__ cell_first,
                            int *__restrict__ fill, int *__restrict__ fill_back, const double *__restrict__ alpha,
                            int *__restrict__ perm, int *__restrict__ inv) {
  int i = blockIdx.x * blockDim.x + threadIdx.x;
  if (i >= n) return;
  const int c = cell_id[i];
  int s;
  if (!fill_back || alpha[i] != 0.0) s = (int)cell_first[c] + atomicAdd(&fill[c], 1);
  else s = (int)cell_first[c + 1] - 1 - atomicAdd(&fill_back[c], 1);
  perm[s] = i;
  inv[i] = s;
}
static __global__ __launch_bounds__(256) void k_cell_sort(long long ncell, const long long *__restrict__ cell_first, const int *__restrict__ npol,
                                                   int *__restrict__ perm, int *__restrict__ inv) {
  const int lane = threadIdx.x & 63;
  const long long c = blockIdx.x * (long long)(blockDim.x >> 6) + (threadIdx.x >> 6);
  if (c >= ncell) return;
  const int a = (int)cell_first[c], b = (int)cell_first[c + 1], m = npol ? a + npol[c] : b;
  for (int part = 0; part < 2; part++) {
    const int lo = part ? m : a, hi = part ? b : m;
    const int cnt = hi - lo;
    if (cnt <= 1) continue;
    if (cnt <= 64) {
      const int v = lane < cnt ? perm[lo + lane] : 0x7fffffff;
      int r = 0;
      for (int k = 0; k < cnt; k++) r += __shfl(v, k, 64) < v;
      __builtin_amdgcn_wave_barrier();
      if (lane < cnt) { perm[lo + r] = v; inv[v] = lo + r; }
    } else if (lane == 0) {
      for (int k = lo + 1; k < hi; k++) {
        const int v = perm[k];
        int j = k - 1;
        while (j >= lo && perm[j] > v) { perm[j + 1] = perm[j]; j--; }
        perm[j + 1] = v;
      }
      for (int k = lo; k < hi; k++) inv[perm[k]] = k;
    }
  }
}
static __global__ void k_map_rows(int n, const int *__restrict__ inv, const int *__restrict__ in, int *__restrict__ out) {
  int i = blockIdx.x * blockDim.x + threadIdx.x;
  if (i < n) out[i] = inv[in[i]];
}
static __global__ void k_map_rows_pad(int n, const int *__restrict__ inv, const int *__restrict__ in, int *__restrict__ out) {
  int i = blockIdx.x * blockDim.x + threadIdx.x;
  if (i < n) out[i] = in[i] >= 0 ? inv[in[i]] : -1;
}
static __global__ void k_slot_from_rows(int n, const int *__restrict__ rows, int *__restrict__ slot) {
  int r = blockIdx.x * blockDim.x + threadIdx.x;
  if (r < n) slot[rows ? rows[r] : r] = r;
}
static __global__ void k_color_map(int n, const int *__restrict__ perm, const int *__restrict__ color_orig, int *__restrict__ color_s) {
  int i = blockIdx.x * blockDim.x + threadIdx.x;
  if (i < n) color_s[i] = color_orig[perm[i]];
}
static __global__ void k_map_range(int lo, int n, const int *__restrict__ inv, int *__restrict__ out) {
  int i = blockIdx.x * blockDim.x + threadIdx.x;
  if (i < n) out[i] = inv[lo + i];
}

__device__ __forceinline__ unsigned color_hash(unsigned x) {
  x ^= x >> 16; x *= 0x7feb352du; x ^= x >> 15; x *= 0x846ca68bu; x ^= x >> 16;
  return x;
}
static __global__ void k_color_adj(int n, const double4 *__restrict__ pos4, const int *__restrict__ perm, int own_lo, int own_hi,
                            Box box, CellGrid g, const long long *__restrict__ cell_first, const int *__restrict__ npol,
                            double colordistsq, int apitch, int *__restrict__ adj, int *__restrict__ deg,
                            unsigned long long *__restrict__ prio, int *__restrict__ color_s, int *__restrict__ flags,
                            int with_halo, int sw) {
  const int i = blockIdx.x * blockDim.x + threadIdx.x;
  if (i >= n) return;
  const double4 ri = pos4[i];
  const int o = perm[i];
  const bool row = __double2loint(ri.w) && o >= own_lo && o < own_hi;
  color_s[i] = -1;
  if (!row) { deg[i] = -1; prio[i] = 0ull; return; }
  int cc[3];
  {
    double fr3[3];
    frac_coords(box, g.lo, ri.x, ri.y, ri.z, fr3);
#pragma unroll
    for (int k = 0; k < 3; k++) {
      double fr = fr3[k];
      fr -= floor(fr);
      int ck = (int)(fr * g.nc[k]);
      cc[k] = ck >= g.nc[k] ? g.nc[k] - 1 : ck;
    }
  }
  int d = 0;
  for (int dz = -sw; dz <= sw; dz++)
    for (int dy = -sw; dy <= sw; dy++)
      for (int dx = -sw; dx <= sw; dx++) {
        int b[3] = {cc[0] + dx, cc[1] + dy, cc[2] + dz};
        bool ok = true;
#pragma unroll
        for (int k = 0; k < 3; k++) {
          if (b[k] < 0 || b[k] >= g.nc[k]) {
            if (!box.periodic[k] || g.nc[k] < 2 * sw + 1) ok = false;
            b[k] = (b[k] + 2 * g.nc[k]) % g.nc[k];
          }
        }
        if (!ok) continue;
        const long long cj = ((long long)b[2] * g.nc[1] + b[1]) * g.nc[0] + b[0];
        const int a = (int)cell_first[cj], e = a + npol[cj];
        for (int j = a; j < e; j++) {
          if (j == i) continue;
          const double4 rj = pos4[j];
          double ex, ey, ez;
          min_image_rint(box, ri.x, ri.y, ri.z, rj.x, rj.y, rj.z, ex, ey, ez);
          if (ex * ex + ey * ey + ez * ez < colordistsq) {
            const int oj = perm[j];
            if (!with_halo && (oj < own_lo || oj >= own_hi)) continue;
            if (d < apitch) adj[(size_t)i * apitch + d] = j;
            d++;
          }
        }
      }
  if (d > apitch) { atomicMax(flags, d); d = apitch; }
  deg[i] = d;
  prio[i] = ((unsigned long long)(d < 255 ? d : 255) << 56) | ((unsigned long long)(color_hash((unsigned)o) >> 8) << 32) | (unsigned)o;
}
static __global__ __launch_bounds__(64) void k_color_cells(int s0, int s1, int s2, int t0, int t1, int t2, int m0, int m1, int m2, int n0, int n1,
                                                    const long long *__restrict__ cell_first, const int *__restrict__ npol, int apitch,
                                                    const int *__restrict__ adj, const int *__restrict__ deg, int *__restrict__ color_s,
                                                    int *__restrict__ flags) {
  const int lane = threadIdx.x;
  const int b = blockIdx.x;
  const int i0 = b % m0, i1 = (b / m0) % m1, i2 = b / (m0 * m1);
  if (i2 >= m2) return;
  const long long c = ((long long)(s2 + t2 * i2) * n1 + (s1 + t1 * i1)) * n0 + (s0 + t0 * i0);
  const int a = (int)cell_first[c], np = npol[c];
  for (int base = 0; base < np; base += 64) {
    const int i = a + base + lane;
    const bool row = base + lane < np && deg[i] >= 0;
    int mine = row ? color_s[i] : 0;
    unsigned long long used = 0ull, inbatch = 0ull;
    int d = 0;
    if (row && mine < 0) {
      d = deg[i];
      for (int k = 0; k < d; k++) {
        const int j = adj[(size_t)i * apitch + k];
        const int cj = color_s[j];
        if (cj >= 0) used |= 1ull << cj;
        const int rel = j - (a + base);
        if (rel >= 0 && rel < 64) inbatch |= 1ull << rel;
      }
    }
    const int todo = __popcll(__ballot(row && mine < 0));
    for (int it = 0; it < todo; it++) {
      const unsigned key = (row && mine < 0) ? (((unsigned)__popcll(used) + 1u) << 16) | ((unsigned)(d < 255 ? d : 255) << 8) | (unsigned)(63 - lane) : 0u;
      unsigned best = key;
#pragma unroll
      for (int o = 32; o > 0; o >>= 1) { const unsigned v = (unsigned)__shfl_xor((int)best, o, 64); best = v > best ? v : best; }
      const int wl = 63 - (int)(best & 63u);
      int cm = 0;
      if (lane == wl) {
        cm = __ffsll((long long)~used) - 1;
// ... 124 lines not shown
  for (int step = 0; step < budget && k >= 0 && k < m; step++) {
    const unsigned long long ek = __shfl(in, k, 64) & ((1ull << k) - 1ull);
    const bool nb = (ek >> lane) & 1ull;
    unsigned long long ok = __shfl(allow, k, 64);
    for (int c = 0; c < top; c++)
      if (((ok >> c) & 1ull) && __ballot(nb && mycol == c)) ok &= ~(1ull << c);
    const int cur = __shfl(mycol, k, 64);
    if (cur >= 0) ok &= ~((2ull << cur) - 1ull);
    if (ok) {
      const int c = __ffsll((long long)ok) - 1;
      if (lane == k) mycol = c;
      k++;
      if (lane == k) mycol = -1;
    } else {
      if (lane == k) mycol = -1;
      k--;
    }
  }
  if (k >= m && lane < m) color_s[ball[lane]] = mycol;
}
static __global__ void k_color_regroup(int n, const int *__restrict__ deg, const int *__restrict__ class_rank, const int *__restrict__ perm,
                                int *__restrict__ color_s, unsigned long long *__restrict__ prio) {
  const int i = blockIdx.x * blockDim.x + threadIdx.x;
  if (i >= n || deg[i] < 0) return;
  const unsigned o = (unsigned)perm[i];
  prio[i] = ((unsigned long long)(63 - class_rank[color_s[i]]) << 56) | ((unsigned long long)(color_hash(o) >> 8) << 32) | o;
  color_s[i] = -1;
}
static __global__ __launch_bounds__(256) void k_color_stats(int n, const int *__restrict__ color_s, const double *__restrict__ rank,
                                                     double *__restrict__ sums, const int *__restrict__ perm, int own_lo, int own_hi) {
  __shared__ double part[128];
  if (threadIdx.x < 128) part[threadIdx.x] = 0.0;
  __syncthreads();
  const int i = blockIdx.x * blockDim.x + threadIdx.x;
  int c = i < n ? color_s[i] : -1;
  if (c >= 0) { const int o = perm[i]; if (o < own_lo || o >= own_hi) c = -1; }
  if (c >= 0) {
    atomicAdd(&part[2 * c], 1.0);
    atomicAdd(&part[2 * c + 1], rank ? rank[i] : 1.0);
  }
  __syncthreads();
  if (threadIdx.x < 128 && part[threadIdx.x] != 0.0) atomicAdd(sums + threadIdx.x, part[threadIdx.x]);
}
static __global__ void k_color_relabel(int n, const int *__restrict__ relabel, const int *__restrict__ perm, int *__restrict__ color_s,
                                int *__restrict__ color_orig) {
  const int i = blockIdx.x * blockDim.x + threadIdx.x;
  if (i >= n) return;
  const int c = color_s[i] >= 0 ? relabel[color_s[i]] : -1;
  color_s[i] = c;
  color_orig[perm[i]] = c;
}
__device__ __forceinline__ int color_class(int j, const int *__restrict__ color_s, const int *__restrict__ perm, int own_lo, int own_hi,
                                           const int *__restrict__ sub, int nsub) {
  const int c = color_s[j];
  if (c < 0) return -1;
  const int o = perm[j];
  if (o < own_lo || o >= own_hi) return -1;
  return sub ? nsub * c + sub[o] : c;
}
static __global__ void k_color_cellcount(long long ncell, int nclass, const long long *__restrict__ cell_first, const int *__restrict__ npol,
                                  const int *__restrict__ color_s, int *__restrict__ cnt, const int *__restrict__ perm, int own_lo, int own_hi,
                                  const int *__restrict__ sub, int nsub) {
  const long long c = blockIdx.x * (long long)blockDim.x + threadIdx.x;
  if (c >= ncell) return;
  const int a = (int)cell_first[c], e = a + npol[c];
  for (int q = 0; q < nclass; q++) {
    int k = 0;
    for (int j = a; j < e; j++) k += color_class(j, color_s, perm, own_lo, own_hi, sub, nsub) == q;
    cnt[(size_t)q * ncell + c] = k;
  }
}
static __global__ void k_color_fill(long long ncell, int nclass, const long long *__restrict__ cell_first, const int *__restrict__ npol,
                             const int *__restrict__ color_s, const int *__restrict__ perm, const long long *__restrict__ off,
                             int *__restrict__ rows_orig, int own_lo, int own_hi, const int *__restrict__ sub, int nsub) {
  const long long c = blockIdx.x * (long long)blockDim.x + threadIdx.x;
  if (c >= ncell) return;
  const int a = (int)cell_first[c], e = a + npol[c];
  for (int q = 0; q < nclass; q++) {
    long long w = off[(size_t)q * ncell + c];
    for (int j = a; j < e; j++) if (color_class(j, color_s, perm, own_lo, own_hi, sub, nsub) == q) rows_orig[w++] = perm[j];
  }
}

template <bool TRI, bool RECHECK>
static __global__ __launch_bounds__(POLAR_BLOCK) void k_nl_build(const int *__restrict__ rows, int nrows,
                                                          const double4 *__restrict__ pos4, Box box, CellGrid g,
                                                          const long long *__restrict__ cell_first, double cutallsq,
                                                          double ddcutsq, long long nl_pitch, long long dd_pitch,
                                                          int *__restrict__ nl_cnt, int *__restrict__ dd_cnt,
                                                          int *__restrict__ nl_j, int *__restrict__ dd_j,
                                                          double *__restrict__ dd_r2, int pad_dd,
                                                          int dd_shift_qm, int dd_pad_index, int *__restrict__ dd_wrap,
                                                          const int *__restrict__ color_s, double colordistsq,
                                                          int *__restrict__ color_conflict,
                                                          const int *__restrict__ dd_slot,
                                                          int *__restrict__ overflow,
                                                          unsigned long long *__restrict__ dd_total) {
  const int dd_shift = dd_shift_qm & 255, dd_qm = dd_shift_qm >> 8;
  const int lane = threadIdx.x & 63;
  const int row = blockIdx.x * POLAR_ROWS_PER_BLOCK + (threadIdx.x >> 6);
  if (row >= nrows) return;
  const int i = rows ? rows[row] : row;
  const double4 ri = pos4[i];
  const int imol = __double2hiint(ri.w), ipol = __double2loint(ri.w);
  const int icol = (RECHECK && color_s && ipol) ? color_s[i] : -2;
  bool clash = RECHECK && color_s && ipol && icol < 0;
  int cc[3];
  double uu[3], edge[3];
  {
    double fr3[3];
    frac_coords(box, g.lo, ri.x, ri.y, ri.z, fr3);
#pragma unroll
    for (int k = 0; k < 3; k++) {
      double fr = fr3[k];
      fr -= floor(fr);
      const double t = fr * g.nc[k];
      int ck = (int)t;
      ck = ck >= g.nc[k] ? g.nc[k] - 1 : ck;
      cc[k] = __builtin_amdgcn_readfirstlane(ck);
      uu[k] = wave_uniform(t - ck); edge[k] = wave_uniform(box.prd[k] / g.nc[k]);
    }
  }
  const int c0 = cc[0], c1 = cc[1], c2 = cc[2];
  const int slot_i = dd_slot ? dd_slot[i] : i;
  const long long nl0 = (long long)i * nl_pitch, dd0 = (long long)(slot_i >= 0 ? slot_i : 0) * dd_pitch;
  int ncount = 0, dcount = 0;
  bool wrap_lane = false;
  const unsigned long long below = (lane == 0) ? 0ull : (~0ull >> (64 - lane));
  const int n0 = g.nc[0], n1 = g.nc[1], n2 = g.nc[2];
  const int zlo = n2 >= 5 ? c2 - 2 : 0, zcnt = n2 >= 5 ? 5 : n2;
  const int ylo = n1 >= 5 ? c1 - 2 : 0, ycnt = n1 >= 5 ? 5 : n1;
  const double reach = sqrt(cutallsq > ddcutsq ? cutallsq : ddcutsq) + 1e-6;
  const double reach2 = wave_uniform(reach * reach);
  const int nsr = zcnt * ycnt;
  int ra0 = 0, rb0 = 0, ra1 = 0, rb1 = 0;
  if (lane < nsr) {
    const int zz = zlo + lane / ycnt, yy = ylo + lane % ycnt;
    int b2 = zz, b1 = yy;
    bool ok = true;
    if (b2 < 0 || b2 >= n2) { if (!box.periodic[2]) ok = false; b2 = (b2 + n2) % n2; }
    if (b1 < 0 || b1 >= n1) { if (!box.periodic[1]) ok = false; b1 = (b1 + n1) % n1; }
    double dzmin = 0.0, dymin = 0.0;
    if (n2 >= 5) { const int d = zz - c2; dzmin = d > 0 ? (d - uu[2]) * edge[2] : (d < 0 ? (uu[2] - (d + 1)) * edge[2] : 0.0); }
    if (n1 >= 5) { const int d = yy - c1; dymin = d > 0 ? (d - uu[1]) * edge[1] : (d < 0 ? (uu[1] - (d + 1)) * edge[1] : 0.0); }
    const double rem2 = reach2 - dzmin * dzmin - dymin * dymin;
    if (g.trim && rem2 < 0.0) ok = false;
    int xlo = n0 >= 5 ? c0 - 2 : 0, xhi = n0 >= 5 ? c0 + 2 : n0 - 1;
    if (ok && g.trim && n0 >= 5) {
      const double xr = sqrt(rem2) / edge[0];
      int lo_off = (int)floor(uu[0] - xr), hi_off = (int)floor(uu[0] + xr);
      lo_off = lo_off < -2 ? -2 : lo_off; hi_off = hi_off > 2 ? 2 : hi_off;
      xlo = c0 + lo_off; xhi = c0 + hi_off;
    }
    if (ok) {
      const long long rowbase = ((long long)b2 * n1 + b1) * n0;
      const int xa = xlo < 0 ? 0 : xlo, xb = xhi >= n0 ? n0 - 1 : xhi;
      ra0 = (int)cell_first[rowbase + xa]; rb0 = (int)cell_first[rowbase + xb + 1];
      if (box.periodic[0]) {
        if (xlo < 0) { ra1 = (int)cell_first[rowbase + xlo + n0]; rb1 = (int)cell_first[rowbase + n0]; }
        else if (xhi >= n0) { ra1 = (int)cell_first[rowbase]; rb1 = (int)cell_first[rowbase + xhi - n0 + 1]; }
      }
    }
  }
  for (int sr = 0; sr < nsr; sr++) {
#pragma unroll
    for (int piece = 0; piece < 2; piece++) {
      const int a = __builtin_amdgcn_readlane(piece ? ra1 : ra0, sr), b = __builtin_amdgcn_readlane(piece ? rb1 : rb0, sr);
      for (int base = a; base < b; base += 64) {
        const int p = base + lane;
        bool in_nl = false, in_dd = false;
        const int j = p;
        int same = 0;
        double rsq = 0.0;
        if (p < b && j != i) {
          const double4 rj = pos4[j];
          double ex, ey, ez;
          const bool shifted = min_image_rint_w<TRI>(box, ri.x, ri.y, ri.z, rj.x, rj.y, rj.z, ex, ey, ez);
          rsq = ex * ex + ey * ey + ez * ez;
          in_nl = rsq <= cutallsq;
          in_dd = ipol && slot_i >= 0 && __double2loint(rj.w) && (rsq < ddcutsq);
          if (RECHECK && icol >= 0 && rsq < colordistsq && __double2loint(rj.w) && color_s[j] == icol) clash = true;
          wrap_lane |= in_dd && shifted;
          same = (imol != 0 && imol == __double2hiint(rj.w)) ? POLAR_NL_SAMEMOL : 0;
        }
        const unsigned long long m_nl = __ballot(in_nl), m_dd = __ballot(in_dd);
        const int kn = ncount + __popcll(m_nl & below), kd = dcount + __popcll(m_dd & below);
        if (in_nl && kn < nl_pitch) nl_j[nl0 + kn] = j | same;
        if (in_dd && kd < dd_pitch) {
          dd_j[dd0 + (dd_shift ? lp_slot(kd, dd_qm) : (long long)kd)] = j << dd_shift;
          if (dd_r2) dd_r2[dd0 + kd] = rsq;
        }
        ncount += __popcll(m_nl);
        dcount += __popcll(m_dd);
      }
    }
  }
  if (pad_dd) {
    const int have = dcount < dd_pitch ? dcount : (int)dd_pitch;
    const int padded = (have + 63) & ~63;
    for (int k = have + lane; k < padded; k += 64) {
      dd_j[dd0 + (dd_shift ? lp_slot(k, dd_qm) : (long long)k)] = (dd_pad_index >= 0 ? dd_pad_index : i) << dd_shift;
      if (dd_r2) dd_r2[dd0 + k] = 1e60;
    }
  }
  if (RECHECK && color_s && __ballot(clash) != 0ull && lane == 0) atomicOr(color_conflict, 1);
  const unsigned long long anywrap = __ballot(wrap_lane);
  if (lane == 0) {
    nl_cnt[i] = ncount; dd_cnt[i] = dcount;
    if (dd_wrap) dd_wrap[i] = anywrap != 0ull;
    if (ncount > nl_pitch || dcount > dd_pitch) atomicMax(overflow, ncount > dcount ? ncount : dcount);
    if (dcount) atomicAdd(dd_total + (blockIdx.x & 63) * 16, (unsigned long long)(dcount < dd_pitch ? dcount : (int)dd_pitch));
  }
}

#ifdef POLAR_LAB
#include "lab/lists_paired_rows.hpp"
#endif

#ifdef POLAR_LAB
#include "lab/lists_cluster_rows.hpp"
#endif

struct LJGrid {
  int nc[3];
  double lo[3], inv[3];
};
__device__ __forceinline__ int lj_cell_of(const LJGrid &g, double x, double y, double z) {
  const double p[3] = {x, y, z};
  int c[3];
#pragma unroll
  for (int k = 0; k < 3; k++) {
    int ck = (int)floor((p[k] - g.lo[k]) * g.inv[k]);
    c[k] = ck < 0 ? 0 : (ck >= g.nc[k] ? g.nc[k] - 1 : ck);
  }
  return (c[2] * g.nc[1] + c[1]) * g.nc[0] + c[0];
}
static __global__ void k_lj_cell_count(int nall, const double *__restrict__ x, LJGrid g, int *__restrict__ cell_id,
                                int *__restrict__ cell_cnt) {
  int i = blockIdx.x * blockDim.x + threadIdx.x;
  if (i >= nall) return;
  const int c = lj_cell_of(g, x[3 * i], x[3 * i + 1], x[3 * i + 2]);
  cell_id[i] = c;
  atomicAdd(&cell_cnt[c], 1);
}
static __global__ void k_lj_cell_fill(int nall, const int *__restrict__ cell_id, const long long *__restrict__ cell_first,
                               int *__restrict__ fill, const double *__restrict__ x, const int *__restrict__ type,
                               const int *__restrict__ mol, const int *__restrict__ tag, double4 *__restrict__ pos,
                               int2 *__restrict__ aux) {
  int i = blockIdx.x * blockDim.x + threadIdx.x;
  if (i >= nall) return;
  const int c = cell_id[i];
  const int s = (int)cell_first[c] + atomicAdd(&fill[c], 1);
  pos[s] = make_double4(x[3 * i], x[3 * i + 1], x[3 * i + 2], __hiloint2double(mol[i], type[i]));
  aux[s] = make_int2(i, tag ? tag[i] : i + 1);
}

static __global__ __launch_bounds__(POLAR_BLOCK) void k_lj_nl_build(int row_lo, int nrows, int ntypes, const double *__restrict__ x,
                                                             const int *__restrict__ type, const int *__restrict__ mol,
                                                             const double4 *__restrict__ pos, const int2 *__restrict__ aux,
                                                             LJGrid g, const long long *__restrict__ cell_first,
                                                             const double *__restrict__ cutneighsq, Box box,
                                                             int exclude_intra, const int *__restrict__ nspecial,
                                                             const int *__restrict__ special, int maxspecial, int sf1,
                                                             int sf2, int sf3, long long pitch, int *__restrict__ cnt,
                                                             int *__restrict__ out_j, int *__restrict__ overflow,
                                                             unsigned long long *__restrict__ total, int typed) {
  extern __shared__ double cn_lds[];
  const int w = ntypes + 1;
  for (int t = threadIdx.x; t < w * w; t += blockDim.x) cn_lds[t] = cutneighsq[t];
  __syncthreads();
  const int lane = threadIdx.x & 63;
  const int r_ = blockIdx.x * POLAR_ROWS_PER_BLOCK + (threadIdx.x >> 6);
  if (r_ >= nrows) return;
  const int i = row_lo + r_;
  const double xi = x[3 * i], yi = x[3 * i + 1], zi = x[3 * i + 2];
  const int itype = type[i], imol = mol[i];
  const double *cn = cn_lds + itype * w;
  int n1 = 0, n2 = 0, n3 = 0;
  if (nspecial) { n1 = nspecial[3 * i]; n2 = nspecial[3 * i + 1]; n3 = nspecial[3 * i + 2]; }
  const int *sp = special ? special + (size_t)i * maxspecial : nullptr;
  const int ci = lj_cell_of(g, xi, yi, zi);
  const int n0 = g.nc[0], n1c = g.nc[1], n2c = g.nc[2];
  const int c0 = ci % n0, c1 = (ci / n0) % n1c, c2 = ci / (n0 * n1c);
  const unsigned long long below = (lane == 0) ? 0ull : (~0ull >> (64 - lane));
  const long long row0 = (long long)i * pitch;
  int count = 0;
  for (int zz = max(c2 - 2, 0); zz <= min(c2 + 2, n2c - 1); zz++)
    for (int yy = max(c1 - 2, 0); yy <= min(c1 + 2, n1c - 1); yy++) {
      const long long rb = ((long long)zz * n1c + yy) * n0;
      const long long a = cell_first[rb + max(c0 - 2, 0)], b = cell_first[rb + min(c0 + 2, n0 - 1) + 1];
      for (long long base = a; base < b; base += 64) {
        const long long p = base + lane;
        bool keep = false;
        int entry = 0;
// ... 168 lines not shown
```

### lammps-induced-dipole-polarization-pair-style_amd/csrc/polar_rows.hpp

```cpp
#pragma once

#include "polar_common.hpp"
#include "polar_force_pair.hpp"
#ifdef POLAR_LAB
#include "lab/force_pair_literal.hpp"
#define POLAR_LIT_PARAM , int literal
#define POLAR_LIT_PASS , literal
#else
#define POLAR_LIT_PARAM
#define POLAR_LIT_PASS
#endif

namespace polar {

static __global__ void k_pack(int n, const int *__restrict__ perm, const double *__restrict__ x, const double *__restrict__ q,
                       const double *__restrict__ alpha, const int *__restrict__ mol, const double *__restrict__ mu0,
                       AtomRec *__restrict__ r0, AtomRec *__restrict__ r1, int *__restrict__ mol_s,
                       double4 *__restrict__ pos4, double4 *__restrict__ xq_s, int wrap, Box box, double lo0, double lo1,
                       double lo2) {
  int i = blockIdx.x * blockDim.x + threadIdx.x;
  if (i == n) {
    AtomRec d;
    d.x = n > 0 ? x[0] : 0.0; d.y = n > 0 ? x[1] : 0.0; d.z = n > 0 ? x[2] : 0.0;
    d.mx = d.my = d.mz = d.q = d.a = 0.0;
    r0[n] = d; r1[n] = d;
  }
  if (i >= n) return;
  const int o = perm ? perm[i] : i;
  AtomRec r;
  r.x = x[3 * o]; r.y = x[3 * o + 1]; r.z = x[3 * o + 2]; r.q = q[o];
  if (wrap) {
    const double lo[3] = {lo0, lo1, lo2};
    double fr[3];
    frac_coords(box, lo, r.x, r.y, r.z, fr);
    const double n2 = box.periodic[2] ? floor(fr[2]) : 0.0, n1 = box.periodic[1] ? floor(fr[1]) : 0.0,
                 n0 = box.periodic[0] ? floor(fr[0]) : 0.0;
    r.z -= n2 * box.prd[2]; r.y -= n2 * box.yz + n1 * box.prd[1]; r.x -= n2 * box.xz + n1 * box.xy + n0 * box.prd[0];
  }
  r.mx = mu0 ? mu0[3 * o] : 0.0; r.my = mu0 ? mu0[3 * o + 1] : 0.0; r.mz = mu0 ? mu0[3 * o + 2] : 0.0;
  r.a = alpha[o];
  r0[i] = r;
  r1[i] = r;
  mol_s[i] = mol[o];
  if (pos4) pos4[i] = make_double4(r.x, r.y, r.z, __hiloint2double(mol[o], r.a != 0.0 ? 1 : 0));
  if (xq_s) xq_s[i] = make_double4(r.x, r.y, r.z, r.q);
}

template <bool ALLPAIRS, int PASS>
static __global__ __launch_bounds__(POLAR_BLOCK) void k_rank(int nlocal, int ntotal, const double *__restrict__ x,
                                                      const double *__restrict__ alpha, const int *__restrict__ mol,
                                                      Box box, RowList nl,
                                                      const int *__restrict__ nl_j,
                                                      const AtomRec *__restrict__ rec,
                                                      const int *__restrict__ mol_s, Scal *scal,
                                                      double *__restrict__ slots,
                                                      double *__restrict__ rank_metric, int nchunk) {
  const int lane = threadIdx.x & 63;
  const int gw = blockIdx.x * POLAR_ROWS_PER_BLOCK + (threadIdx.x >> 6);
  if (gw >= nlocal * nchunk) return;
  const int i = gw % nlocal, chunk = gw / nlocal;
  const double xi = ALLPAIRS ? x[3 * i] : rec[i].x, yi = ALLPAIRS ? x[3 * i + 1] : rec[i].y,
               zi = ALLPAIRS ? x[3 * i + 2] : rec[i].z, ai = ALLPAIRS ? alpha[i] : rec[i].a;
  const int mi = ALLPAIRS ? mol[i] : mol_s[i];
  double rmin = (PASS == 1) ? 1000.0 : __longlong_as_double((long long)scal->rmin_bits);
  double rmin2 = 1.0e6;
  const double far2 = (rmin * 1.5) * (rmin * 1.5) * 1.000001;
  double acc = 0.0;
  long long beg = 0, end = ntotal;
  if (!ALLPAIRS) row_range(nl, i, beg, end);
  else if (nchunk > 1) { const long long per = ((ntotal + nchunk - 1) / nchunk + 255) / 256 * 256; beg = chunk * per; end = beg + per < ntotal ? beg + per : ntotal; }
  constexpr int U = ALLPAIRS ? 4 : 1;
  for (long long base = beg; base < end; base += 64 * U) {
    double px[U], py[U], pz[U], pa[U];
    int pj[U], pm[U];
#pragma unroll
    for (int u = 0; u < U; u++) {
      const long long p = base + 64 * u + lane;
      pj[u] = i;
      if (p < end) pj[u] = ALLPAIRS ? (int)p : (nl_j[p] & POLAR_NL_MASK);
      if (ALLPAIRS) {
        px[u] = x[3 * pj[u]]; py[u] = x[3 * pj[u] + 1]; pz[u] = x[3 * pj[u] + 2];
        pa[u] = alpha[pj[u]]; pm[u] = mol[pj[u]];
      } else {
        const AtomRec rj = rec[pj[u]];
        px[u] = rj.x; py[u] = rj.y; pz[u] = rj.z; pa[u] = rj.a; pm[u] = mol_s[pj[u]];
      }
    }
#pragma unroll
    for (int u = 0; u < U; u++) {
      bool hit = false;
      double term = 0.0;
      if (pj[u] != i) {
        double dx, dy, dz;
        if (ALLPAIRS) { dx = xi - px[u]; dy = yi - py[u]; dz = zi - pz[u]; }
        else min_image_rint(box, xi, yi, zi, px[u], py[u], pz[u], dx, dy, dz);
        const double rsq = dx * dx + dy * dy + dz * dz;
        const bool molok = (mi != pm[u]) || mi == 0;
        if (PASS == 1) {
          if (ai > 0 && pa[u] > 0 && molok) rmin2 = fmin(rmin2, rsq);
        } else if (rsq < far2 && molok && rmin * 1.5 > sqrt(rsq)) {
          hit = true;
          term = ai * pa[u];
        }
      }
      if (PASS == 2) {
        unsigned long long m = __ballot(hit);
        while (m) {
          const int b = __ffsll((long long)m) - 1;
          acc += __shfl(term, b, 64);
          m &= m - 1;
        }
      }
    }
  }
  if (PASS == 1) {
    rmin = wave_min(fmin(rmin, sqrt(rmin2)));
    if (lane == 0)
      atomicMin((unsigned long long *)slot_ptr(slots, SL_RMIN), (unsigned long long)__double_as_longlong(rmin));
  } else {
    if (lane == 0) rank_metric[i] = acc;
  }
}

static __global__ __launch_bounds__(POLAR_BLOCK) void k_rank_order(int n, const double *__restrict__ rk, int *__restrict__ order, int *__restrict__ pos) {
  const int lane = threadIdx.x & 63;
  const int i = blockIdx.x * POLAR_ROWS_PER_BLOCK + (threadIdx.x >> 6);
  if (i >= n) return;
// ... 518 lines not shown
```

### lammps-induced-dipole-polarization-pair-style_amd/csrc/polar_step.hip

```cpp
#include "polar_handle.hpp"

void launch_scan(long long n, const int *in, long long *out, DBuf<long long> &tot, hipStream_t s) {
  const int nb = (int)std::max<long long>(1, (n + POLAR_SCAN_ITEMS - 1) / POLAR_SCAN_ITEMS);
  tot.ensure((size_t)nb + 1);
  k_scan_block<<<nb, 1024, 0, s>>>(n, in, out, tot.p);
  if (nb > 1) {
    k_scan_totals<<<1, 1024, 0, s>>>(nb, tot.p, out + n);
    k_scan_add<<<nblk(n - POLAR_SCAN_ITEMS, 256), 256, 0, s>>>(n, out, tot.p);
  }
}

void build_cells(polar_handle *h) {
  const polar_settings &st = h->ph.st;
  const int n = h->nlocal;
  const double cutall = std::max(st.cut_coul, st.dd_cutoff);
  double width[3];
  box_widths(h->box, width);
  for (int k = 0; k < 3; k++)
    if (h->box.periodic[k] && width[k] < 2.0 * cutall * (1.0 - 1e-12))
      throw InputError("dd_cutoff mode needs box lengths >= 2*max(cut_coul,dd_cutoff); use exact mode (dd_cutoff 0)");
  CellGrid &g = h->grid;
  g.trim = 1;
#ifdef POLAR_LAB
  if (const char *e = getenv("POLAR_NL_TRIM")) g.trim = atoi(e);
#endif
  if (h->box.triclinic) g.trim = 0;
  long long ncell = 1;
  for (int k = 0; k < 3; k++) {
    g.nc[k] = std::max(1, (int)std::floor(width[k] / (0.5 * cutall)));
    if (h->sweep_kernel == 4 && k == 0 && h->tile_wide) g.nc[k] = std::max(1, (int)std::floor(width[k] / cutall));
    if (h->sweep_kernel == 4 && h->box.periodic[k] && g.nc[k] >= 7 && (g.nc[k] & 1)) g.nc[k] -= 1;
    h->tile_sw[k] = std::max(1, std::min(2, (int)std::ceil(st.dd_cutoff / (width[k] / g.nc[k]) - 1e-9)));
    g.lo[k] = h->boxlo[k];
    g.inv[k] = g.nc[k] / h->box.prd[k];
    ncell *= g.nc[k];
  }
  h->ncell = ncell;
  if (h->sweep_kernel == 4) {
    struct Cls { int start, stride, count; };
    std::vector<Cls> cls[3];
    for (int k = 0; k < 3; k++) {
      const int nc = g.nc[k];
      const bool seam = h->box.periodic[k] && (nc & 1) && nc > 1;
      const int lim = seam ? nc - 1 : nc;
      if ((lim + 1) / 2 > 0) cls[k].push_back(Cls{0, 2, (lim + 1) / 2});
      if (lim / 2 > 0) cls[k].push_back(Cls{1, 2, lim / 2});
      if (seam) cls[k].push_back(Cls{nc - 1, 1, 1});
    }
    h->tile_launches.clear();
    for (const Cls &cz : cls[2]) for (const Cls &cy : cls[1]) for (const Cls &cx : cls[0]) {
      TileLaunch L;
      L.start[0] = cx.start; L.stride[0] = cx.stride; L.count[0] = cx.count;
      L.start[1] = cy.start; L.stride[1] = cy.stride; L.count[1] = cy.count;
      L.start[2] = cz.start; L.stride[2] = cz.stride; L.count[2] = cz.count;
      for (int k = 0; k < 3; k++) L.nc[k] = g.nc[k];
      h->tile_launches.push_back(L);
    }
    for (int k = 0; k < 3; k++) { h->tile_all.start[k] = 0; h->tile_all.stride[k] = 1; h->tile_all.count[k] = g.nc[k]; h->tile_all.nc[k] = g.nc[k]; }
  }
  hipStream_t s = h->stream;
  h->d_cell_id.ensure(n); h->d_cell_cnt.ensure(ncell + 1); h->d_cell_fill.ensure(2 * (ncell + 1));
  h->d_cell_first.ensure(ncell + 2); h->d_perm.ensure(n + 1); h->d_inv.ensure(n + 1);
  zero_many(s, {{h->d_cell_cnt.p, (size_t)(ncell + 1) * sizeof(int)}, {h->d_cell_fill.p, 2 * (size_t)(ncell + 1) * sizeof(int)}});
  k_cell_count<<<nblk(n, 256), 256, 0, s>>>(n, h->d_x.p, g, h->box, h->d_cell_id.p, h->d_cell_cnt.p);
  launch_scan(ncell, h->d_cell_cnt.p, h->d_cell_first.p, h->d_scan_a, s);
  k_cell_fill<<<nblk(n, 256), 256, 0, s>>>(n, h->d_cell_id.p, h->d_cell_first.p, h->d_cell_fill.p,
                                           (h->pol_first || h->sweep_kernel == 4) ? h->d_cell_fill.p + ncell + 1 : nullptr, h->d_alpha.p, h->d_perm.p, h->d_inv.p);
  k_cell_sort<<<nblk(ncell, 4), 256, 0, s>>>(ncell, h->d_cell_first.p, (h->pol_first || h->sweep_kernel == 4) ? h->d_cell_fill.p : nullptr, h->d_perm.p, h->d_inv.p);
  h->sorted = true;
  if (sharded(h)) {
    h->d_ownrows.ensure(own_n(h) + 1);
    k_map_range<<<nblk(own_n(h), 256), 256, 0, s>>>(own_lo(h), own_n(h), h->d_inv.p, h->d_ownrows.p);
  }
}

void compute_slots(polar_handle *h) {
  const polar_settings &st = h->ph.st;
  const bool gs = st.polar_gs || st.polar_gs_ranked;
  const int n = h->nlocal;
  hipStream_t s = h->stream;
  h->d_slot.ensure(n + 1);
  HIPCHECK(hipMemsetAsync(h->d_slot.p, 0xFF, (size_t)(n + 1) * sizeof(int), s));
  if (gs && h->colors_valid) {
    const int tot = h->color_off.empty() ? 0 : h->color_off.back();
    if (tot > 0) k_slot_from_rows<<<nblk(tot, 256), 256, 0, s>>>(tot, h->d_rows.p, h->d_slot.p);
    h->slots_by_color = true;
    h->slots_epoch = h->color_epoch;
  } else {
    k_slot_from_rows<<<nblk(own_n(h), 256), 256, 0, s>>>(own_n(h), own_rows(h), h->d_slot.p);
    h->slots_by_color = false;
  }
}

void build_lists(polar_handle *h) {
  const polar_settings &st = h->ph.st;
  const int n = h->nlocal;
  const double cutall = std::max(st.cut_coul, st.dd_cutoff);
  hipStream_t s = h->stream;
  const CellGrid &g = h->grid;
  if (h->nl_pitch == 0 && getenv("POLAR_INIT_PITCH")) h->nl_pitch = h->dd_pitch = ((std::max(64, atoi(getenv("POLAR_INIT_PITCH"))) + 63) / 64) * 64;
  if (h->nl_pitch == 0) {
    double vol = h->box.prd[0] * h->box.prd[1] * h->box.prd[2];
    {
      int nc[3];
      long long tot = 1;
      for (int k = 0; k < 3; k++) { nc[k] = std::max(1, std::min(64, (int)(h->box.prd[k] / cutall))); tot *= nc[k]; }
      std::vector<char> occ((size_t)tot, 0);
      for (int a = 0; a < n; a++) {
        long long c = 0, mul = 1;
        for (int k = 0; k < 3; k++) {
          double fr = (h->hx[3 * (size_t)a + k] - h->grid.lo[k]) / h->box.prd[k];
          fr -= std::floor(fr);
          c += mul * std::min(nc[k] - 1, (int)(fr * nc[k]));
          mul *= nc[k];
        }
        occ[(size_t)c] = 1;
      }
      long long filled = 0;
      for (char v : occ) filled += v;
      if (filled > 0) vol *= (double)filled / (double)tot;
    }
    h->dens = n / vol;
    double mean = n / vol * 4.18879020478639 * cutall * cutall * cutall;
    h->nl_pitch = h->dd_pitch = (((long long)(1.5 * mean) + 64) / 64 + 1) * 64;
  }
  if (h->sweep_kernel == 2) h->dd_pitch = ((h->dd_pitch + 255) / 256) * 256;
  if ((h->sweep_kernel == 2 || h->sweep_kernel == 3) && ((long long)n + 1) * (long long)sizeof(AtomRec) >= (1ll << 31))
    throw InputError("more than 2^25 atoms on one handle: the 32-bit record offsets of the sweep's index stream would wrap (shard the system)");
  h->d_nl_cnt.ensure(n + 1); h->d_dd_cnt.ensure(n + 1);
  h->d_nl_j.ensure((size_t)n * h->nl_pitch + 64);
  if (h->sweep_kernel < 3) h->d_dd_j.ensure((size_t)n * h->dd_pitch + 1024);
  else h->d_dd_j.ensure(64);
  int mode = h->cache_r2;
  if (h->sweep_kernel == 1) mode = 0;
  if (h->sweep_kernel == 2) mode = 3;
  if (h->sweep_kernel >= 3) mode = 4;
  if (mode < 0) {
    const double est_pairs = h->dd_pairs > 0 ? (double)h->dd_pairs : 0.35 * (double)own_n(h) * (double)h->dd_pitch;
    mode = (12.0 * est_pairs < 200.0e6) ? 1 : 2;
  }
  h->stream_mode = mode;
  const bool r2c = mode == 1;
  if (mode == 1) h->d_dd_r2.ensure((size_t)n * h->dd_pitch + 64);
  else if (mode == 0) h->d_dd_s.ensure((size_t)n * h->dd_pitch + 64);
  double *r2p = r2c ? h->d_dd_r2.p : nullptr;
  double2 *sp = mode == 0 ? h->d_dd_s.p : nullptr;
  bool fuse = mode != 0 && mode != 4;
#ifdef POLAR_LAB
  if (getenv("POLAR_NO_FUSE_R2")) fuse = false;
#endif
  const double cutallsq = cutall * cutall, ddsq = mode == 4 ? -1.0 : st.dd_cutoff * st.dd_cutoff;
  const int nr = own_n(h);
  const int *rows = own_rows(h);
  zero_many(s, {{h->d_nl_cnt.p, (size_t)(n + 1) * sizeof(int)}, {h->d_dd_cnt.p, (size_t)(n + 1) * sizeof(int)},
                {h->d_overflow.p, 16 * sizeof(int)}, {h->d_ddtot.p, 64 * 16 * sizeof(unsigned long long)}});
  const bool lp = mode == 3;
  if (lp) h->d_dd_wrap.ensure(n + 1);
  const bool recheck = h->colors_valid && h->colors_recheck && h->sweep_kernel < 3 && (int)h->h_color.size() == n;
  if (h->colors_recheck && !recheck) { h->colors_valid = false; h->colors_recheck = false; }
  if (recheck) {
    h->d_color_s.ensure(n + 1);
    k_color_map<<<nblk(n, 256), 256, 0, s>>>(n, h->d_perm.p, h->d_color_orig.p, h->d_color_s.p);
  }
#define NLB(TRI, RC)                                                                                                          \
  k_nl_build<TRI, RC><<<nblk(nr, POLAR_ROWS_PER_BLOCK), POLAR_BLOCK, 0, s>>>(                                                 \
      rows, nr, h->d_pos4.p, h->box, g, h->d_cell_first.p, cutallsq, ddsq, h->nl_pitch, h->dd_pitch, h->d_nl_cnt.p,            \
      h->d_dd_cnt.p, h->d_nl_j.p, h->d_dd_j.p, fuse ? r2p : nullptr, fuse ? 1 : 0, lp ? (6 | (h->lp_quad_major << 8)) : 0,    \
      lp ? n : -1, lp ? h->d_dd_wrap.p : nullptr, recheck ? h->d_color_s.p : nullptr, h->color_keep * h->color_keep,           \
      h->d_overflow.p + 8, lp ? h->d_slot.p : nullptr, h->d_overflow.p, h->d_ddtot.p)
  if (h->box.triclinic) { if (recheck) NLB(true, true); else NLB(true, false); }
  else                  { if (recheck) NLB(false, true); else NLB(false, false); }
#undef NLB
  const RowList ddl{h->d_dd_cnt.p, h->dd_pitch};
  if (fuse || mode == 4) {
  }
#ifdef POLAR_LAB
  else if (st.damping_type == POLAR_DAMP_EXPONENTIAL)
    k_dd_scalars<0><<<nblk(nr, POLAR_ROWS_PER_BLOCK), POLAR_BLOCK, 0, s>>>(rows, nr, h->d_rec0.p, h->box, ddl, h->d_dd_j.p, st.polar_damp, sp, r2p);
  else
    k_dd_scalars<1><<<nblk(nr, POLAR_ROWS_PER_BLOCK), POLAR_BLOCK, 0, s>>>(rows, nr, h->d_rec0.p, h->box, ddl, h->d_dd_j.p, st.polar_damp, sp, r2p);
#endif
  HIPCHECK(hipMemcpyAsync(h->h_flags, h->d_overflow.p, sizeof(int), hipMemcpyDeviceToHost, s));
  HIPCHECK(hipMemcpyAsync(h->h_ddtot, h->d_ddtot.p, 64 * 16 * sizeof(unsigned long long), hipMemcpyDeviceToHost, s));
}
template <bool AP>
static void launch_rank(polar_handle *h, int pass) {
  const int n = h->nlocal, ntot = h->nlocal + h->nghost;
  dim3 grid(nblk(n, POLAR_ROWS_PER_BLOCK)), block(POLAR_BLOCK);
  if (pass == 2) k_fold_scal<<<1, POLAR_NSLOT, 0, h->stream>>>(h->d_scal.p, h->d_slots.p, 1);
  const int nchunk = (AP && pass == 1) ? std::max(1, std::min(16, 8192 / std::max(n, 1))) : 1;
  if (pass == 1)
    k_rank<AP, 1><<<nblk((long long)n * nchunk, POLAR_ROWS_PER_BLOCK), block, 0, h->stream>>>(n, ntot, h->d_x.p, h->d_alpha.p, h->d_mol.p, h->box, RowList{h->d_nl_cnt.p, h->nl_pitch},
                                                 h->d_nl_j.p, h->d_rec0.p, h->d_mol_s.p, h->d_scal.p, h->d_slots.p, h->d_rank.p, nchunk);
  else
    k_rank<AP, 2><<<grid, block, 0, h->stream>>>(n, ntot, h->d_x.p, h->d_alpha.p, h->d_mol.p, h->box, RowList{h->d_nl_cnt.p, h->nl_pitch},
                                                 h->d_nl_j.p, h->d_rec0.p, h->d_mol_s.p, h->d_scal.p, h->d_slots.p, h->d_rank.p, 1);
}

void launch_rank_pass(polar_handle *h, bool allpairs, int pass) {
  if (allpairs) launch_rank<true>(h, pass); else launch_rank<false>(h, pass);
}

template <bool AP, int DAMP, int EP>
void launch_field(polar_handle *h, int nrows, const int *rows) {
  const polar_settings &st = h->ph.st;
  if (nrows <= 0) return;
  const int fb = h->field_block;
  const size_t lds = AP ? 0 : (size_t)(fb / 64) * 64 * 5 * sizeof(double2);
  k_field<AP, DAMP, EP><<<nblk(nrows, fb / 64), fb, lds, h->stream>>>(
      nrows, rows, h->nlocal, h->d_rec0.p, h->d_rec1.p, h->box, RowList{h->d_dd_cnt.p, h->dd_pitch}, h->d_dd_j.p, h->d_dd_s.p,
      st.dd_cutoff * st.dd_cutoff, st.polar_damp, h->d_ef_s.p, h->d_F.p, h->d_scal.p, h->d_slots.p
#ifdef POLAR_LAB
      , h->ablate
#endif
      );
}
template <int EP>
void launch_field_dyn(polar_handle *h, bool ap, int nrows, const int *rows) {
  const bool expd = h->ph.st.damping_type == POLAR_DAMP_EXPONENTIAL;
  if (ap) { if (expd) launch_field<true, 0, EP>(h, nrows, rows); else launch_field<true, 1, EP>(h, nrows, rows); }
#ifdef POLAR_LAB
  else    { if (expd) launch_field<false, 0, EP>(h, nrows, rows); else launch_field<false, 1, EP>(h, nrows, rows); }
#else
  else throw std::logic_error("k_field's list branch exists in the lab build only");
#endif
}

#ifdef POLAR_LAB
#include "lab/launch_quad.inc"
#else
template <int EP> inline void launch_field_quad(polar_handle *, int, const int *) { throw std::logic_error("lab build only"); }
#endif

void prepare_lp(polar_handle *h) {
  const polar_settings &st = h->ph.st;
  const bool gs = st.polar_gs || st.polar_gs_ranked;
  const int tot = gs ? (h->color_off.empty() ? 0 : h->color_off.back()) : own_n(h);
  h->d_lpdesc.ensure((size_t)tot + 1);
  h->lp_npart = 0;
  if (deterministic(h)) {
    h->d_lp_pend.ensure(4 * (size_t)tot + 4);
    const int nlaunch = gs ? (int)h->color_off.size() - 1 : 1;
    h->lp_npart = tot / 256 + nlaunch + 1;
    h->d_lp_part.ensure((size_t)h->lp_npart + 1);
    HIPCHECK(hipMemsetAsync(h->d_lp_part.p, 0, (size_t)h->lp_npart * sizeof(double), h->stream));
  }
  if (tot > 0)
    k_lp_desc<<<nblk(tot, 256), 256, 0, h->stream>>>(tot, gs ? h->d_rows.p : own_rows(h), RowList{h->d_dd_cnt.p, h->dd_pitch},
                                                     h->d_dd_wrap.p, h->d_lpdesc.p);
}
template <int EP>
void launch_field_lp(polar_handle *h, int nrows, const int2 *desc) {
  const long long row0 = desc - h->d_lpdesc.p;
  if (nrows <= 0) return;
// ... 623 lines not shown
  HIPCHECK(hipEventRecord(h->ev[4], s));
  if (lj_late) launch_lj();
}

int phase_finish(polar_handle *h, polar_result *out) {
  const polar_settings &st = h->ph.st;
  const int n = h->nlocal, nall = h->nlocal + h->nghost;
  const bool ap = !(st.dd_cutoff > 0.0);
  const bool expd = st.damping_type == POLAR_DAMP_EXPONENTIAL;
  const int eflag = h->step_eflag, vmode = h->step_vflag % 4;
  hipStream_t s = h->stream;
#ifdef POLAR_LAB
  if (!ap && h->sweep_kernel == 4 && !st.zodid)
    k_srec_unpack<<<nblk(n, 256), 256, 0, s>>>(n, h->d_scal.p, h->d_srec0.p, h->d_srec1.p, h->d_rec0.p, h->d_rec1.p);
#endif
  k_fallback<<<nblk(n, 256), 256, 0, s>>>(n, h->d_scal.p, h->d_rec0.p, h->d_rec1.p, h->d_ef_s.p);
  HIPCHECK(hipEventRecord(h->ev[5], s));
  k_unpack<<<nblk(n, 256), 256, 0, s>>>(n, h->sorted ? h->d_perm.p : nullptr, h->d_scal.p, h->d_rec0.p, h->d_rec1.p, h->d_ef_s.p, h->d_mu.p, h->d_ef.p);
  if (h->early_mu && n > 0) {
    HIPCHECK(hipEventRecord(h->ev_mu_ready, s));
    HIPCHECK(hipStreamWaitEvent(h->dl_stream, h->ev_mu_ready, 0));
    HIPCHECK(hipMemcpyAsync(h->early_mu, h->d_mu.p, 3 * (size_t)n * sizeof(double), hipMemcpyDeviceToHost, h->dl_stream));
    if (h->early_ef) HIPCHECK(hipMemcpyAsync(h->early_ef, h->d_ef.p, 3 * (size_t)n * sizeof(double), hipMemcpyDeviceToHost, h->dl_stream));
    HIPCHECK(hipEventRecord(h->ev_dl1, h->dl_stream));
  }
  double *vatom = (h->step_vflag / 4) ? h->d_vatom.p : nullptr;
  auto join_lj = [&]() { if (h->lj_forked) { HIPCHECK(hipStreamWaitEvent(s, h->ev_join, 0)); h->lj_forked = false; } };
  if (vatom) join_lj();
  const bool split_f = h->full_list && vmode == 2;
  double *fdst = h->d_f.p;
  if (split_f) {
    h->d_fpol.ensure(3 * (size_t)n + 3);
    HIPCHECK(hipMemsetAsync(h->d_fpol.p, 0, 3 * (size_t)n * sizeof(double), s));
    fdst = h->d_fpol.p;
  }
  if (ap) { if (expd) launch_force<true, 0>(h, eflag, vmode == 1, vatom, fdst); else launch_force<true, 1>(h, eflag, vmode == 1, vatom, fdst); }
  else    { if (expd) launch_force<false, 0>(h, eflag, vmode == 1, vatom, fdst); else launch_force<false, 1>(h, eflag, vmode == 1, vatom, fdst); }
  join_lj();
  if (split_f) {
    k_virial_fdotr<<<std::min(1024, nblk(n, 256)), 256, 0, s>>>(n, h->d_x.p, h->d_fpol.p, h->d_slots.p);
    k_add_into<<<nblk(3 * (long long)n, 256), 256, 0, s>>>(3 * (long long)n, h->d_fpol.p, h->d_f.p);
  } else if (vmode == 2) k_virial_fdotr<<<std::min(1024, nblk(nall, 256)), 256, 0, s>>>(nall, h->d_x.p, h->d_f.p, h->d_slots.p);
  if (ewald_on(h)) ewald_forces(h);
  k_fold_scal<<<1, POLAR_NSLOT, 0, s>>>(h->d_scal.p, h->d_slots.p, 0);
  HIPCHECK(hipEventRecord(h->ev[6], s));
  if (h->early_mu && h->user_mu && n > 0) {
    HIPCHECK(hipEventSynchronize(h->ev_dl1));
    const double *sm = h->early_mu, *se = h->early_ef;
    double *um = h->user_mu, *ue = h->user_ef;
    host_chunks(3 * (size_t)n, [&](size_t a, size_t b) {
      memcpy(um + a, sm + a, (b - a) * sizeof(double));
      if (ue && se) memcpy(ue + a, se + a, (b - a) * sizeof(double));
    });
  }
  read_scal(h);
  h->mu_resident = true;
  h->mu_host_in_sync = false;

  const Scal &sc = *h->h_scal;
  out->eng_vdwl = sc.eng_vdwl; out->eng_coul = sc.eng_coul;
  out->u_self = sc.u_self; out->u_ef = sc.u_ef; out->u_dd = sc.u_dd;
  out->eng_pol = sc.u_self + sc.u_ef + sc.u_dd;
  for (int k = 0; k < 6; k++) out->virial[k] = sc.virial[k];
  if (ewald_on(h)) {
    double ew[7];
    HIPCHECK(hipMemcpyAsync(ew, h->d_ew_out.p, sizeof(ew), hipMemcpyDeviceToHost, h->stream));
    HIPCHECK(hipStreamSynchronize(h->stream));
    if (eflag) { out->u_ef = ew[0]; out->eng_pol = sc.u_self + ew[0] + sc.u_dd; }
    if (vmode) for (int k = 0; k < 6; k++) out->virial[k] += ew[1 + k];
    float a = 0.f, b = 0.f;
    HIPCHECK(hipEventElapsedTime(&a, h->ev_ks[0], h->ev_ks[1]));
    HIPCHECK(hipEventElapsedTime(&b, h->ev_ks[2], h->ev_ks[3]));
    out->ms_kspace = (double)a + (double)b;
    out->nkvec = h->ew_nk;
  }
  long long rb = (long long)sc.rmin_bits;
  memcpy(&out->rmin, &rb, sizeof(double));
  out->rms_dmu = std::sqrt(std::max(0.0, sc.last_change));
  h->ntrace = std::min(h->ntrace, sc.sweeps);
  out->iterations = sc.iterations; out->sweeps = sc.sweeps; out->status = sc.status ? POLAR_WARN_NOT_CONVERGED : POLAR_OK;
  h->last_sweeps = (!st.fixed_iteration && !st.zodid && !sc.status && sc.done) ? sc.sweeps : 0;
  if (!ap) {
    unsigned long long tot = 0;
    for (int k = 0; k < 64; k++) tot += h->h_ddtot[16 * k];
    h->dd_pairs = (long long)tot;
  }
  out->dd_pairs = ap ? (long long)n * (n - 1) : h->dd_pairs;
  out->ms_color_host = h->ms_color_host;
  h->ms_color_host = 0.0;
  float ms;
  auto el = [&](int a, int b) { HIPCHECK(hipEventElapsedTime(&ms, h->ev[a], h->ev[b])); return (double)ms; };
  out->ms_list = el(0, 1); out->ms_rank = el(1, 2); out->ms_static = el(3, 4);
  HIPCHECK(hipEventElapsedTime(&ms, h->ev_lj0, h->ev_lj1));
  out->ms_ljcoul = ms;
  out->ms_solve = el(4, 5); out->ms_force = el(5, 6); out->ms_total = el(0, 6);
  if (sc.status) h->warn = "Number of iterations exceeding max_iterations, setting dipoles to alpha*E";
  return out->status;
}

void clear_flags(polar_handle *h) { for (int k = 0; k < 16; k++) h->h_flags[k] = 0; }
void tile_fallback(polar_handle *h) {
  h->sweep_kernel = 2;
  h->colors_valid = false; h->slots_by_color = false;
  h->nl_pitch = h->dd_pitch = 0;
  h->warn = "tile sweep unavailable for this system (cell neighbourhood beyond the LDS, or a cell beyond the builder's limits): row sweep in use";
}
bool grow_pitches(polar_handle *h) {
  bool again = false;
  if (h->h_flags[0] != 0) {
    const long long need = ((long long)(1.25 * h->h_flags[0]) / 64 + 1) * 64;
    h->nl_pitch = h->dd_pitch = std::max(need, h->nl_pitch + 64);
    again = true;
  }
  if (h->h_flags[4] != 0) { h->cl_pitch = (((long long)(1.25 * h->h_flags[4]) + 255) / 256) * 256; again = true; }
  if (h->sweep_kernel == 4) {
    if (h->h_flags[7] != 0) { tile_fallback(h); return true; }
    if (h->h_flags[5] != 0) {
      const int need = (int)(((long long)(1.15 * h->h_flags[5]) + 16 + 63) / 64 * 64);
      if (need > tile_lds_cap()) { tile_fallback(h); return true; }
      h->un_pitch = std::max(h->un_pitch, need); h->un_lds = h->un_pitch;
      again = true;
    }
    if (h->h_flags[6] != 0) { h->pitch16 = ((long long)(1.25 * h->h_flags[6]) + 511) / 512 * 512; again = true; }
    if (!again && h->h_flags[9] > 0) {
      h->tile_max_u = h->h_flags[9];
      h->un_lds = std::min(h->un_pitch, (int)((long long)(1.06 * (h->tile_max_u + 1)) + 8 + 7) / 8 * 8);
      if (getenv("POLAR_DEBUG") && !h->tile_reported) {
        h->tile_reported = true;
        fprintf(stderr, "[polar] tile sweep: %lld cells (%d x %d x %d), %d launches per sweep, largest union %d records, union pitch %d, "
                "LDS request %zu bytes (%d records), row pitch %lld entries\n", h->ncell, h->grid.nc[0], h->grid.nc[1], h->grid.nc[2],
                (int)h->tile_launches.size(), h->tile_max_u, h->un_pitch, tile_lds_bytes(std::min(h->un_pitch, h->un_lds)), h->un_lds, h->pitch16);
      }
    }
  }
  return again;
}

int do_compute(polar_handle *h, int eflag, int vflag, const double *mu_host, polar_result *out) {
  memset(out, 0, sizeof(*out));
  const bool ap = !(h->ph.st.dd_cutoff > 0.0);
  int rc = 0;
  bool done = false;
  struct Attempt { polar_handle *h; ~Attempt() { h->attempt = 0; } } guard{h};
  for (int attempt = 0; attempt < 5; attempt++) {
    clear_flags(h);
    h->attempt = attempt;
    try {
      phase_begin(h, eflag, vflag, mu_host);
    } catch (const TileUnavailable &) {
      tile_fallback(h);
      continue;
    }
    if (!h->ph.st.zodid) solve(h, ap, out);
    const int nc = out->ncolors;
    rc = phase_finish(h, out);
    out->ncolors = nc;
    if (ap || !grow_pitches(h)) { done = true; break; }
    memset(out, 0, sizeof(*out));
  }
  if (!done) throw std::runtime_error("neighbor list pitch overflow persists");
  return rc;
}

void step_begin_lists(polar_handle *h, int eflag, int vflag) {
  HIPCHECK(hipSetDevice(h->device));
  clear_flags(h);
  try {
// ... 21 lines not shown
```

Before: 16.29 million.

## Skip per-pair minimum-image rint in neighbor build using per-stripe periodic shifts

Adds a uniform-shift path to the neighbor-list build kernel. Each atom gets an 'outside the primary box' flag, and each cell stripe gets a precomputed periodic shift code. For rows and wavefronts where no atom is outside the box, the pair displacement is a plain subtraction plus a constant shift instead of a per-pair minimum-image rint. The change also moves loop-invariant quantities (reach, cell edge) to the host, uses readfirstlane/mbcnt for wave-uniform values and compaction, and adds trip counters and a debug list-download API. The trip counters cost an extra atomic per row, and computing the outside flag adds work when positions are packed.

```diff
diff --git a/include/polar_mi355x.h b/include/polar_mi355x.h
--- a/include/polar_mi355x.h
+++ b/include/polar_mi355x.h
@@ -118,6 +118,7 @@
 int polar_compute_resident(polar_handle *h, int eflag, int vflag, polar_result *out);
 void *polar_dev_ptr(polar_handle *h, const char *name);
 int polar_download(polar_handle *h, const char *name, double *dst, long long n);
+int polar_debug_lists(polar_handle *h, const char *name, int *dst, long long n);
 int polar_upload_mu(polar_handle *h, const double *mu, long long n);
 
 
diff --git a/lammps-induced-dipole-polarization-pair-style_amd/__init__.py b/lammps-induced-dipole-polarization-pair-style_amd/__init__.py
--- a/lammps-induced-dipole-polarization-pair-style_amd/__init__.py
+++ b/lammps-induced-dipole-polarization-pair-style_amd/__init__.py
@@ -120,6 +120,7 @@
     "polar_compute_resident": (C.c_int, [C.c_void_p, C.c_int, C.c_int, C.POINTER(Result)]),
     "polar_dev_ptr": (C.c_void_p, [C.c_void_p, C.c_char_p]),
     "polar_download": (C.c_int, [C.c_void_p, C.c_char_p, _dp, C.c_longlong]),
+    "polar_debug_lists": (C.c_int, [C.c_void_p, C.c_char_p, _ip, C.c_longlong]),
     "polar_upload_mu": (C.c_int, [C.c_void_p, _dp, C.c_longlong]),
     "polar_set_stream": (C.c_int, [C.c_void_p, C.c_void_p]),
     "polar_set_row_range": (C.c_int, [C.c_void_p, C.c_int, C.c_int]),
@@ -458,6 +459,16 @@
         nc = self._ck(self.L.polar_get_colors(self.h, a.ctypes.data_as(C.POINTER(C.c_int)), n))
         return nc, a
 
+    def debug_lists(self, name):
+        n = self._ck(self.L.polar_debug_lists(self.h, name.encode(), None, 0))
+        a = np.zeros(max(n, 1), dtype=np.int32)
+        self._ck(self.L.polar_debug_lists(self.h, name.encode(), a.ctypes.data_as(_ip), n))
+        if name == "info":
+            v = a[:16].view(np.int64)
+            return dict(nlocal=int(v[0]), nl_pitch=int(v[1]), dd_pitch=int(v[2]), uniform=bool(v[3]), trips_uniform=int(v[4]),
+                        trips_rint=int(v[5]), lp=bool(v[6] & 1), quad_major=bool(v[6] & 2), rows=int(v[7]))
+        return a[:n]
+
     def download(self, name, n):
         a = np.zeros(n)
         self._ck(self.L.polar_download(self.h, name.encode(), _dptr(a), n))
diff --git a/lammps-induced-dipole-polarization-pair-style_amd/csrc/lab/lists_cluster_rows.hpp b/lammps-induced-dipole-polarization-pair-style_amd/csrc/lab/lists_cluster_rows.hpp
--- a/lammps-induced-dipole-polarization-pair-style_amd/csrc/lab/lists_cluster_rows.hpp
+++ b/lammps-induced-dipole-polarization-pair-style_amd/csrc/lab/lists_cluster_rows.hpp
@@ -98,7 +98,7 @@
         int hits = 0;
         if (j < b && j != m0 && j != m1 && j != m2 && j != m3) {
           const double4 rj = pos4[j];
-          if (__double2loint(rj.w)) {
+          if (__double2loint(rj.w) & POLAR_POS_POL) {
 #pragma unroll
             for (int k = 0; k < 4; k++) {
               double ex, ey, ez;
diff --git a/lammps-induced-dipole-polarization-pair-style_amd/csrc/lab/lists_paired_rows.hpp b/lammps-induced-dipole-polarization-pair-style_amd/csrc/lab/lists_paired_rows.hpp
--- a/lammps-induced-dipole-polarization-pair-style_amd/csrc/lab/lists_paired_rows.hpp
+++ b/lammps-induced-dipole-polarization-pair-style_amd/csrc/lab/lists_paired_rows.hpp
@@ -90,7 +90,7 @@
         bool inA = false, inB = false;
         if (j < b) {
           const double4 rj = pos4[j];
-          if (__double2loint(rj.w)) {
+          if (__double2loint(rj.w) & POLAR_POS_POL) {
             double ex, ey, ez;
             const bool shA = min_image_rint_w<TRI>(box, rA.x, rA.y, rA.z, rj.x, rj.y, rj.z, ex, ey, ez);
             inA = j != iA && ex * ex + ey * ey + ez * ez < ddcutsq;
diff --git a/lammps-induced-dipole-polarization-pair-style_amd/csrc/polar_api.hip b/lammps-induced-dipole-polarization-pair-style_amd/csrc/polar_api.hip
--- a/lammps-induced-dipole-polarization-pair-style_amd/csrc/polar_api.hip
+++ b/lammps-induced-dipole-polarization-pair-style_amd/csrc/polar_api.hip
@@ -187,6 +187,7 @@
     for (auto &e : h->ev_ks) HIPCHECK(hipEventCreate(&e));
     HIPCHECK(hipStreamCreateWithFlags(&h->dl_stream, hipStreamNonBlocking));
     if (getenv("POLAR_NO_OVERLAP")) h->overlap_lj = false;
+    if (const char *e = getenv("POLAR_NL_GENERIC")) h->nl_generic = atoi(e) != 0;
     if (const char *e = getenv("POLAR_LJ_PERS")) h->lj_pers = atoi(e);
     if (const char *e = getenv("POLAR_LJ_PERS_THREADS")) h->lj_pers_threads = std::max(256, std::min(POLAR_LJ_PERS_THREADS, (atoi(e) / 64) * 64));
     { int ncu = 0; if (hipDeviceGetAttribute(&ncu, hipDeviceAttributeMultiprocessorCount, device) == hipSuccess) h->ncu = ncu; }
@@ -744,6 +745,40 @@
     return POLAR_OK;
   });
 }
+int polar_debug_lists(polar_handle *h, const char *name, int *dst, long long n) {
+  long long have = -1;
+  int rc = guarded(h, [&]() {
+    need_device(h);
+    if (!name) throw InputError("polar_debug_lists: null name");
+    const long long na = h->nlocal;
+    if (strcmp(name, "info") == 0) {
+      const long long info[8] = {na, h->nl_pitch, h->dd_pitch, h->nl_uniform ? 1 : 0, h->nl_trips_uniform, h->nl_trips_rint,
+                                 (h->sweep_kernel == 2 ? 1 : 0) | (h->lp_quad_major ? 2 : 0), own_n(h)};
+      have = 16;
+      if (dst && n >= have) memcpy(dst, info, sizeof(info));
+      return (int)POLAR_OK;
+    }
+    if (h->nl_pitch <= 0 || !h->d_nl_cnt.p) throw InputError("polar_debug_lists: no list-mode compute has run on this handle");
+    const bool lp = h->sweep_kernel == 2;
+    const int *src = nullptr;
+    if (strcmp(name, "nl_cnt") == 0) { src = h->d_nl_cnt.p; have = na; }
+    else if (strcmp(name, "dd_cnt") == 0) { src = h->d_dd_cnt.p; have = na; }
+    else if (strcmp(name, "nl_j") == 0) { src = h->d_nl_j.p; have = na * h->nl_pitch; }
+    else if (strcmp(name, "dd_j") == 0 && h->sweep_kernel < 3) { src = h->d_dd_j.p; have = na * h->dd_pitch; }
+    else if (strcmp(name, "dd_wrap") == 0 && lp) { src = h->d_dd_wrap.p; have = na; }
+    else if (strcmp(name, "dd_slot") == 0 && lp) { src = h->d_slot.p; have = na; }
+    else if (strcmp(name, "perm") == 0) { src = h->d_perm.p; have = na; }
+    else throw InputError("polar_debug_lists: unknown array name");
+    if (dst && n >= have && have > 0) {
+      HIPCHECK(hipSetDevice(h->device));
+      HIPCHECK(hipStreamSynchronize(h->stream));
+      HIPCHECK(hipMemcpy(dst, src, (size_t)have * sizeof(int), hipMemcpyDeviceToHost));
+    }
+    return (int)POLAR_OK;
+  });
+  if (rc < 0) return rc;
+  return have > 2147483647LL ? POLAR_ERR_INPUT : (int)have;
+}
 int polar_upload_mu(polar_handle *h, const double *mu, long long n) {
   return guarded(h, [&]() {
     need_device(h);
diff --git a/lammps-induced-dipole-polarization-pair-style_amd/csrc/polar_common.hpp b/lammps-induced-dipole-polarization-pair-style_amd/csrc/polar_common.hpp
--- a/lammps-induced-dipole-polarization-pair-style_amd/csrc/polar_common.hpp
+++ b/lammps-induced-dipole-polarization-pair-style_amd/csrc/polar_common.hpp
@@ -222,6 +222,8 @@
 
 #define POLAR_NL_SAMEMOL 0x40000000
 #define POLAR_NL_MASK 0x3FFFFFFF
+#define POLAR_POS_POL 1
+#define POLAR_POS_OUTSIDE 2
 
 struct RecQuad { double2 a, b, c, d; };
 __device__ __forceinline__ RecQuad fetch_records(const AtomRec *__restrict__ rec, int j, double2 *stage, int lane) {
diff --git a/lammps-induced-dipole-polarization-pair-style_amd/csrc/polar_handle.hpp b/lammps-induced-dipole-polarization-pair-style_amd/csrc/polar_handle.hpp
--- a/lammps-induced-dipole-polarization-pair-style_amd/csrc/polar_handle.hpp
+++ b/lammps-induced-dipole-polarization-pair-style_amd/csrc/polar_handle.hpp
@@ -271,6 +271,9 @@
   double *early_mu = nullptr, *early_ef = nullptr, *user_mu = nullptr, *user_ef = nullptr;
   hipEvent_t ev_fchunk[4] = {nullptr, nullptr, nullptr, nullptr};
   bool overlap_lj = true;
+  bool nl_generic = false;
+  bool nl_uniform = false;
+  long long nl_trips_uniform = 0, nl_trips_rint = 0;
   bool lj_forked = false;
   std::vector<double> h_tmp;
   double *h_stage = nullptr;
diff --git a/lammps-induced-dipole-polarization-pair-style_amd/csrc/polar_lists.hpp b/lammps-induced-dipole-polarization-pair-style_amd/csrc/polar_lists.hpp
--- a/lammps-induced-dipole-polarization-pair-style_amd/csrc/polar_lists.hpp
+++ b/lammps-induced-dipole-polarization-pair-style_amd/csrc/polar_lists.hpp
@@ -8,6 +8,7 @@
   int trim;
   int nc[3];
   double lo[3], inv[3];
+  double edge[3];
 };
 
 __device__ __forceinline__ int cell_of(const CellGrid &g, const Box &b, double x, double y, double z) {
@@ -178,7 +179,7 @@
   if (i >= n) return;
   const double4 ri = pos4[i];
   const int o = perm[i];
-  const bool row = __double2loint(ri.w) && o >= own_lo && o < own_hi;
+  const bool row = (__double2loint(ri.w) & POLAR_POS_POL) && o >= own_lo && o < own_hi;
   color_s[i] = -1;
   if (!row) { deg[i] = -1; prio[i] = 0ull; return; }
   int cc[3];
@@ -469,11 +470,13 @@
   }
 }
 
-template <bool TRI, bool RECHECK>
+struct alignas(32) PosRec { double x, y, z; int w, mol; };
+static_assert(sizeof(PosRec) == sizeof(double4), "PosRec overlays a double4");
+template <bool TRI, bool RECHECK, bool UNI>
 static __global__ __launch_bounds__(POLAR_BLOCK) void k_nl_build(const int *__restrict__ rows, int nrows,
                                                           const double4 *__restrict__ pos4, Box box, CellGrid g,
                                                           const long long *__restrict__ cell_first, double cutallsq,
-                                                          double ddcutsq, long long nl_pitch, long long dd_pitch,
+                                                          double ddcutsq, double reach2, long long nl_pitch, long long dd_pitch,
                                                           int *__restrict__ nl_cnt, int *__restrict__ dd_cnt,
                                                           int *__restrict__ nl_j, int *__restrict__ dd_j,
                                                           double *__restrict__ dd_r2, int pad_dd,
@@ -488,8 +491,11 @@
   const int row = blockIdx.x * POLAR_ROWS_PER_BLOCK + (threadIdx.x >> 6);
   if (row >= nrows) return;
   const int i = rows ? rows[row] : row;
-  const double4 ri = pos4[i];
-  const int imol = __double2hiint(ri.w), ipol = __double2loint(ri.w);
+  const PosRec *__restrict__ const prec = reinterpret_cast<const PosRec *>(pos4);
+  const PosRec ri = prec[i];
+  const int iw = __builtin_amdgcn_readfirstlane(ri.w);
+  const int imol = __builtin_amdgcn_readfirstlane(ri.mol), ipol = iw & POLAR_POS_POL;
+  const bool row_rint = !UNI || (iw & POLAR_POS_OUTSIDE) != 0;
   const int icol = (RECHECK && color_s && ipol) ? color_s[i] : -2;
   bool clash = RECHECK && color_s && ipol && icol < 0;
   int cc[3];
@@ -505,28 +511,35 @@
       int ck = (int)t;
       ck = ck >= g.nc[k] ? g.nc[k] - 1 : ck;
       cc[k] = __builtin_amdgcn_readfirstlane(ck);
-      uu[k] = wave_uniform(t - ck); edge[k] = wave_uniform(box.prd[k] / g.nc[k]);
+      uu[k] = wave_uniform(t - ck); edge[k] = g.edge[k];
     }
   }
   const int c0 = cc[0], c1 = cc[1], c2 = cc[2];
-  const int slot_i = dd_slot ? dd_slot[i] : i;
+  const int slot_i = __builtin_amdgcn_readfirstlane(dd_slot ? dd_slot[i] : i);
   const long long nl0 = (long long)i * nl_pitch, dd0 = (long long)(slot_i >= 0 ? slot_i : 0) * dd_pitch;
+  int *__restrict__ const nl_row = nl_j + nl0, *__restrict__ const ddj_row = dd_j + dd0;
+  const int nlp = nl_pitch < 0x7fffffffll ? (int)nl_pitch : 0x7fffffff, ddp = dd_pitch < 0x7fffffffll ? (int)dd_pitch : 0x7fffffff;
+  const bool dd_row = ipol && slot_i >= 0;
+  const unsigned long long dd_mask = dd_row ? ~0ull : 0ull;
+  const int same_bit = imol != 0 ? POLAR_NL_SAMEMOL : 0;
+  const int self_base = i - lane;
   int ncount = 0, dcount = 0;
   bool wrap_lane = false;
-  const unsigned long long below = (lane == 0) ? 0ull : (~0ull >> (64 - lane));
   const int n0 = g.nc[0], n1 = g.nc[1], n2 = g.nc[2];
   const int zlo = n2 >= 5 ? c2 - 2 : 0, zcnt = n2 >= 5 ? 5 : n2;
   const int ylo = n1 >= 5 ? c1 - 2 : 0, ycnt = n1 >= 5 ? 5 : n1;
-  const double reach = sqrt(cutallsq > ddcutsq ? cutallsq : ddcutsq) + 1e-6;
-  const double reach2 = wave_uniform(reach * reach);
   const int nsr = zcnt * ycnt;
   int ra0 = 0, rb0 = 0, ra1 = 0, rb1 = 0;
+  int scode = 0;
   if (lane < nsr) {
-    const int zz = zlo + lane / ycnt, yy = ylo + lane % ycnt;
+    const int ymul = ycnt == 5 ? 13108 : (ycnt == 4 ? 16384 : (ycnt == 3 ? 21846 : (ycnt == 2 ? 32768 : 65536)));
+    const int zq = (lane * ymul) >> 16;
+    const int zz = zlo + zq, yy = ylo + (lane - zq * ycnt);
     int b2 = zz, b1 = yy;
     bool ok = true;
-    if (b2 < 0 || b2 >= n2) { if (!box.periodic[2]) ok = false; b2 = (b2 + n2) % n2; }
-    if (b1 < 0 || b1 >= n1) { if (!box.periodic[1]) ok = false; b1 = (b1 + n1) % n1; }
+    if (UNI) scode = (zz < 0 ? 16 : (zz >= n2 ? 32 : 0)) | (yy < 0 ? 4 : (yy >= n1 ? 8 : 0));
+    if (b2 < 0 || b2 >= n2) { if (!box.periodic[2]) ok = false; b2 += b2 < 0 ? n2 : -n2; }
+    if (b1 < 0 || b1 >= n1) { if (!box.periodic[1]) ok = false; b1 += b1 < 0 ? n1 : -n1; }
     double dzmin = 0.0, dymin = 0.0;
     if (n2 >= 5) { const int d = zz - c2; dzmin = d > 0 ? (d - uu[2]) * edge[2] : (d < 0 ? (uu[2] - (d + 1)) * edge[2] : 0.0); }
     if (n1 >= 5) { const int d = yy - c1; dymin = d > 0 ? (d - uu[1]) * edge[1] : (d < 0 ? (uu[1] - (d + 1)) * edge[1] : 0.0); }
@@ -534,7 +547,7 @@
     if (g.trim && rem2 < 0.0) ok = false;
     int xlo = n0 >= 5 ? c0 - 2 : 0, xhi = n0 >= 5 ? c0 + 2 : n0 - 1;
     if (ok && g.trim && n0 >= 5) {
-      const double xr = sqrt(rem2) / edge[0];
+      const double xr = sqrt(rem2) * g.inv[0];
       int lo_off = (int)floor(uu[0] - xr), hi_off = (int)floor(uu[0] + xr);
       lo_off = lo_off < -2 ? -2 : lo_off; hi_off = hi_off > 2 ? 2 : hi_off;
       xlo = c0 + lo_off; xhi = c0 + hi_off;
@@ -544,37 +557,53 @@
       const int xa = xlo < 0 ? 0 : xlo, xb = xhi >= n0 ? n0 - 1 : xhi;
       ra0 = (int)cell_first[rowbase + xa]; rb0 = (int)cell_first[rowbase + xb + 1];
       if (box.periodic[0]) {
-        if (xlo < 0) { ra1 = (int)cell_first[rowbase + xlo + n0]; rb1 = (int)cell_first[rowbase + n0]; }
-        else if (xhi >= n0) { ra1 = (int)cell_first[rowbase]; rb1 = (int)cell_first[rowbase + xhi - n0 + 1]; }
+        if (xlo < 0) { ra1 = (int)cell_first[rowbase + xlo + n0]; rb1 = (int)cell_first[rowbase + n0]; if (UNI) scode |= 1; }
+        else if (xhi >= n0) { ra1 = (int)cell_first[rowbase]; rb1 = (int)cell_first[rowbase + xhi - n0 + 1]; if (UNI) scode |= 2; }
       }
     }
   }
+  int trips_uni = 0, trips_rint = 0;
   for (int sr = 0; sr < nsr; sr++) {
+    const int sc = UNI ? __builtin_amdgcn_readlane(scode, sr) : 0;
+    const double sy = (sc & 4) ? box.prd[1] : ((sc & 8) ? -box.prd[1] : 0.0), sz = (sc & 16) ? box.prd[2] : ((sc & 32) ? -box.prd[2] : 0.0);
 #pragma unroll
     for (int piece = 0; piece < 2; piece++) {
       const int a = __builtin_amdgcn_readlane(piece ? ra1 : ra0, sr), b = __builtin_amdgcn_readlane(piece ? rb1 : rb0, sr);
+      const double sx = !piece ? 0.0 : ((sc & 1) ? box.prd[0] : ((sc & 2) ? -box.prd[0] : 0.0));
+      const bool run_shifted = (sc >> 2) != 0 || (piece && (sc & 3) != 0);
       for (int base = a; base < b; base += 64) {
-        const int p = base + lane;
-        bool in_nl = false, in_dd = false;
-        const int j = p;
-        int same = 0;
-        double rsq = 0.0;
-        if (p < b && j != i) {
-          const double4 rj = pos4[j];
-          double ex, ey, ez;
-          const bool shifted = min_image_rint_w<TRI>(box, ri.x, ri.y, ri.z, rj.x, rj.y, rj.z, ex, ey, ez);
-          rsq = ex * ex + ey * ey + ez * ez;
-          in_nl = rsq <= cutallsq;
-          in_dd = ipol && slot_i >= 0 && __double2loint(rj.w) && (rsq < ddcutsq);
-          if (RECHECK && icol >= 0 && rsq < colordistsq && __double2loint(rj.w) && color_s[j] == icol) clash = true;
-          wrap_lane |= in_dd && shifted;
-          same = (imol != 0 && imol == __double2hiint(rj.w)) ? POLAR_NL_SAMEMOL : 0;
+        const int p = base + lane, j = p;
+        const bool act = p < b && base != self_base;
+        const PosRec rj = prec[(unsigned)(p < b ? p : b - 1)];
+        const int jw = rj.w;
+        double ex, ey, ez;
+        bool shifted;
+        if (UNI && !row_rint && __builtin_amdgcn_ballot_w64((jw & POLAR_POS_OUTSIDE) != 0) == 0ull) {
+          ex = ri.x - rj.x; ey = ri.y - rj.y; ez = ri.z - rj.z;
+          if (piece) ex += sx;
+          ey += sy; ez += sz;
+          shifted = run_shifted;
+          trips_uni++;
+        } else {
+          shifted = min_image_rint_w<TRI>(box, ri.x, ri.y, ri.z, rj.x, rj.y, rj.z, ex, ey, ez);
+          trips_rint++;
         }
-        const unsigned long long m_nl = __ballot(in_nl), m_dd = __ballot(in_dd);
-        const int kn = ncount + __popcll(m_nl & below), kd = dcount + __popcll(m_dd & below);
-        if (in_nl && kn < nl_pitch) nl_j[nl0 + kn] = j | same;
-        if (in_dd && kd < dd_pitch) {
-          dd_j[dd0 + (dd_shift ? lp_slot(kd, dd_qm) : (long long)kd)] = j << dd_shift;
+        const double rsq = ex * ex + ey * ey + ez * ez;
+        const bool jpol = (jw & POLAR_POS_POL) != 0;
+        const bool c_nl = rsq <= cutallsq, c_dd = rsq < ddcutsq;
+        const bool in_nl = act && c_nl;
+        const bool in_dd = act && dd_row && jpol && c_dd;
+        if (RECHECK && act && icol >= 0 && rsq < colordistsq && jpol && color_s[j] == icol) clash = true;
+        wrap_lane |= in_dd && shifted;
+        const int same = rj.mol == imol ? same_bit : 0;
+        const unsigned long long m_act = __builtin_amdgcn_ballot_w64(p < b) & __builtin_amdgcn_ballot_w64(base != self_base);
+        const unsigned long long m_nl = m_act & __builtin_amdgcn_ballot_w64(c_nl);
+        const unsigned long long m_dd = m_act & __builtin_amdgcn_ballot_w64(jpol) & __builtin_amdgcn_ballot_w64(c_dd) & dd_mask;
+        const int kn = (int)__builtin_amdgcn_mbcnt_hi((unsigned)(m_nl >> 32), __builtin_amdgcn_mbcnt_lo((unsigned)m_nl, (unsigned)ncount));
+        const int kd = (int)__builtin_amdgcn_mbcnt_hi((unsigned)(m_dd >> 32), __builtin_amdgcn_mbcnt_lo((unsigned)m_dd, (unsigned)dcount));
+        if (in_nl && kn < nlp) nl_row[(unsigned)kn] = j | same;
+        if (in_dd && kd < ddp) {
+          ddj_row[(dd_shift ? (unsigned)lp_slot(kd, dd_qm) : (unsigned)kd)] = j << dd_shift;
           if (dd_r2) dd_r2[dd0 + kd] = rsq;
         }
         ncount += __popcll(m_nl);
@@ -597,6 +626,7 @@
     if (dd_wrap) dd_wrap[i] = anywrap != 0ull;
     if (ncount > nl_pitch || dcount > dd_pitch) atomicMax(overflow, ncount > dcount ? ncount : dcount);
     if (dcount) atomicAdd(dd_total + (blockIdx.x & 63) * 16, (unsigned long long)(dcount < dd_pitch ? dcount : (int)dd_pitch));
+    atomicAdd(dd_total + (blockIdx.x & 63) * 16 + 1, (unsigned long long)trips_uni | ((unsigned long long)trips_rint << 32));
   }
 }
 
diff --git a/lammps-induced-dipole-polarization-pair-style_amd/csrc/polar_rows.hpp b/lammps-induced-dipole-polarization-pair-style_amd/csrc/polar_rows.hpp
--- a/lammps-induced-dipole-polarization-pair-style_amd/csrc/polar_rows.hpp
+++ b/lammps-induced-dipole-polarization-pair-style_amd/csrc/polar_rows.hpp
@@ -42,7 +42,15 @@
   r0[i] = r;
   r1[i] = r;
   mol_s[i] = mol[o];
-  if (pos4) pos4[i] = make_double4(r.x, r.y, r.z, __hiloint2double(mol[o], r.a != 0.0 ? 1 : 0));
+  if (pos4) {
+    const double lo[3] = {lo0, lo1, lo2};
+    double fr[3];
+    frac_coords(box, lo, r.x, r.y, r.z, fr);
+    bool outside = false;
+#pragma unroll
+    for (int k = 0; k < 3; k++) outside |= box.periodic[k] && floor(fr[k]) != 0.0;
+    pos4[i] = make_double4(r.x, r.y, r.z, __hiloint2double(mol[o], (r.a != 0.0 ? POLAR_POS_POL : 0) | (outside ? POLAR_POS_OUTSIDE : 0)));
+  }
   if (xq_s) xq_s[i] = make_double4(r.x, r.y, r.z, r.q);
 }
 
diff --git a/lammps-induced-dipole-polarization-pair-style_amd/csrc/polar_step.hip b/lammps-induced-dipole-polarization-pair-style_amd/csrc/polar_step.hip
--- a/lammps-induced-dipole-polarization-pair-style_amd/csrc/polar_step.hip
+++ b/lammps-induced-dipole-polarization-pair-style_amd/csrc/polar_step.hip
@@ -33,6 +33,7 @@
     h->tile_sw[k] = std::max(1, std::min(2, (int)std::ceil(st.dd_cutoff / (width[k] / g.nc[k]) - 1e-9)));
     g.lo[k] = h->boxlo[k];
     g.inv[k] = g.nc[k] / h->box.prd[k];
+    g.edge[k] = h->box.prd[k] / g.nc[k];
     ncell *= g.nc[k];
   }
   h->ncell = ncell;
@@ -150,6 +151,7 @@
   if (getenv("POLAR_NO_FUSE_R2")) fuse = false;
 #endif
   const double cutallsq = cutall * cutall, ddsq = mode == 4 ? -1.0 : st.dd_cutoff * st.dd_cutoff;
+  const double reach = std::sqrt(std::max(cutallsq, ddsq)) + 1e-6, reach2 = reach * reach;
   const int nr = own_n(h);
   const int *rows = own_rows(h);
   zero_many(s, {{h->d_nl_cnt.p, (size_t)(n + 1) * sizeof(int)}, {h->d_dd_cnt.p, (size_t)(n + 1) * sizeof(int)},
@@ -162,14 +164,18 @@
     h->d_color_s.ensure(n + 1);
     k_color_map<<<nblk(n, 256), 256, 0, s>>>(n, h->d_perm.p, h->d_color_orig.p, h->d_color_s.p);
   }
-#define NLB(TRI, RC)                                                                                                          \
-  k_nl_build<TRI, RC><<<nblk(nr, POLAR_ROWS_PER_BLOCK), POLAR_BLOCK, 0, s>>>(                                                 \
-      rows, nr, h->d_pos4.p, h->box, g, h->d_cell_first.p, cutallsq, ddsq, h->nl_pitch, h->dd_pitch, h->d_nl_cnt.p,            \
+#define NLB(TRI, RC, UNI)                                                                                                     \
+  k_nl_build<TRI, RC, UNI><<<nblk(nr, POLAR_ROWS_PER_BLOCK), POLAR_BLOCK, 0, s>>>(                                            \
+      rows, nr, h->d_pos4.p, h->box, g, h->d_cell_first.p, cutallsq, ddsq, reach2, h->nl_pitch, h->dd_pitch, h->d_nl_cnt.p,    \
       h->d_dd_cnt.p, h->d_nl_j.p, h->d_dd_j.p, fuse ? r2p : nullptr, fuse ? 1 : 0, lp ? (6 | (h->lp_quad_major << 8)) : 0,    \
       lp ? n : -1, lp ? h->d_dd_wrap.p : nullptr, recheck ? h->d_color_s.p : nullptr, h->color_keep * h->color_keep,           \
       h->d_overflow.p + 8, lp ? h->d_slot.p : nullptr, h->d_overflow.p, h->d_ddtot.p)
-  if (h->box.triclinic) { if (recheck) NLB(true, true); else NLB(true, false); }
-  else                  { if (recheck) NLB(false, true); else NLB(false, false); }
+  bool uni = !h->nl_generic && !h->box.triclinic && h->color_keep <= cutall;
+  for (int k = 0; k < 3; k++) if (h->box.periodic[k] && g.nc[k] < 6) uni = false;
+  h->nl_uniform = uni;
+  if (h->box.triclinic) { if (recheck) NLB(true, true, false); else NLB(true, false, false); }
+  else if (uni)         { if (recheck) NLB(false, true, true); else NLB(false, false, true); }
+  else                  { if (recheck) NLB(false, true, false); else NLB(false, false, false); }
 #undef NLB
   const RowList ddl{h->d_dd_cnt.p, h->dd_pitch};
   if (fuse || mode == 4) {
@@ -959,7 +965,13 @@
   h->last_sweeps = (!st.fixed_iteration && !st.zodid && !sc.status && sc.done) ? sc.sweeps : 0;
   if (!ap) {
     unsigned long long tot = 0;
-    for (int k = 0; k < 64; k++) tot += h->h_ddtot[16 * k];
+    unsigned long long trips = 0;
+    h->nl_trips_uniform = h->nl_trips_rint = 0;
+    for (int k = 0; k < 64; k++) {
+      tot += h->h_ddtot[16 * k];
+      trips = h->h_ddtot[16 * k + 1];
+      h->nl_trips_uniform += (long long)(trips & 0xFFFFFFFFull); h->nl_trips_rint += (long long)(trips >> 32);
+    }
     h->dd_pairs = (long long)tot;
   }
   out->dd_pairs = ap ? (long long)n * (n - 1) : h->dd_pairs;
```

Measured after the change: 16.26 million. No clear change (-0.2%).
